# tczhangzhi/pytorch-distributed

Measured on AMD Instinct MI355X. Metric: ImageNet images/sec (ResNet-50 train step, whole job), higher is better.
Workload: dtype bf16; 1 GPU; model=resnet50, global_batch=3072, image_size=224, parallelism=dp1, style=ddp, hip_ext=True, hipgraph=False

## Files before the change

### amdtrain/models/resnet.py

```python

from __future__ import annotations

from typing import Callable, Dict, List, Optional, Type, Union

import torch
import torch.nn as nn

from ..ops import fused as OF


import os

from ..ops.conv import AmdConv2d, GradCell, ResidualGradTap
from ..ops.linear import AmdLinear


def _residual_fuse_enabled() -> bool:
    return os.environ.get("AMDTRAIN_RESFUSE", "1") == "1"


def conv3x3(in_planes: int, out_planes: int, stride: int = 1,
            groups: int = 1) -> nn.Conv2d:
    return AmdConv2d(in_planes, out_planes, kernel_size=3, stride=stride,
                     padding=1, groups=groups, bias=False)


def conv1x1(in_planes: int, out_planes: int, stride: int = 1) -> nn.Conv2d:
    return AmdConv2d(in_planes, out_planes, kernel_size=1, stride=stride,
                     bias=False)


class FusedBatchNorm2d(nn.BatchNorm2d):

    def forward(self, x: torch.Tensor) -> torch.Tensor:
        return OF.batch_norm(x, self, relu=False)

    def forward_relu(self, x: torch.Tensor) -> torch.Tensor:
        return OF.batch_norm(x, self, relu=True)


class BasicBlock(nn.Module):
    expansion = 1

    def __init__(self, inplanes: int, planes: int, stride: int = 1,
                 downsample: Optional[nn.Module] = None):
        super().__init__()
        self.conv1 = conv3x3(inplanes, planes, stride)
        self.bn1 = FusedBatchNorm2d(planes)
        self.relu = nn.ReLU(inplace=True)
        self.conv2 = conv3x3(planes, planes)
        self.bn2 = FusedBatchNorm2d(planes)
        self.downsample = downsample
        self.stride = stride

    def forward(self, x: torch.Tensor) -> torch.Tensor:
        identity = x
        cell = None
        if (self.training and x.is_cuda and torch.is_grad_enabled()
                and _residual_fuse_enabled()):
            cell = getattr(x, "_amdtrain_next_cell", None)
        out = self.bn1.forward_relu(self.conv1(x))
        out = self.conv2(out)
        if cell is not None:
            cell.armed = True
            tapped = ResidualGradTap.apply(x, cell)
            identity = self.downsample(tapped)                 if self.downsample is not None else tapped
        elif self.downsample is not None:
            identity = self.downsample(x)
        return OF.bn_add_relu(out, self.bn2, identity)


class Bottleneck(nn.Module):
    expansion = 4

    def __init__(self, inplanes: int, planes: int, stride: int = 1,
                 downsample: Optional[nn.Module] = None, groups: int = 1,
                 base_width: int = 64):
        super().__init__()
        width = int(planes * (base_width / 64.0)) * groups
        self.conv1 = conv1x1(inplanes, width)
        self.bn1 = FusedBatchNorm2d(width)
        self.conv2 = conv3x3(width, width, stride, groups)
        self.bn2 = FusedBatchNorm2d(width)
        self.conv3 = conv1x1(width, planes * self.expansion)
        self.bn3 = FusedBatchNorm2d(planes * self.expansion)
        self.relu = nn.ReLU(inplace=True)
        self.downsample = downsample
        self.stride = stride

    def forward(self, x: torch.Tensor) -> torch.Tensor:
        identity = x
        cell = None
        if (self.training and x.is_cuda and torch.is_grad_enabled()
                and _residual_fuse_enabled()):
            cell = getattr(x, "_amdtrain_next_cell", None)
        out = self.bn1.forward_relu(self.conv1(x))
        out = self.bn2.forward_relu(self.conv2(out))
        out = self.conv3(out)
        if cell is not None:
            cell.armed = True
            tapped = ResidualGradTap.apply(x, cell)
            identity = self.downsample(tapped)                 if self.downsample is not None else tapped
        elif self.downsample is not None:
            identity = self.downsample(x)
        return OF.bn_add_relu(out, self.bn3, identity)


class ResNet(nn.Module):
    def __init__(self, block: Type[Union[BasicBlock, Bottleneck]],
                 layers: List[int], num_classes: int = 1000,
                 zero_init_residual: bool = False, groups: int = 1,
                 width_per_group: int = 64):
        super().__init__()
        self.groups = groups
        self.base_width = width_per_group
        self.inplanes = 64
        self.conv1 = AmdConv2d(3, 64, kernel_size=7, stride=2, padding=3,
                               bias=False)
        self.bn1 = FusedBatchNorm2d(64)
        self.relu = nn.ReLU(inplace=True)
        self.maxpool = nn.MaxPool2d(kernel_size=3, stride=2, padding=1)
        self.layer1 = self._make_layer(block, 64, layers[0])
        self.layer2 = self._make_layer(block, 128, layers[1], stride=2)
        self.layer3 = self._make_layer(block, 256, layers[2], stride=2)
        self.layer4 = self._make_layer(block, 512, layers[3], stride=2)
        self.avgpool = nn.AdaptiveAvgPool2d((1, 1))
        self.fc = AmdLinear(512 * block.expansion, num_classes)

        for m in self.modules():
            if isinstance(m, nn.Conv2d):
                nn.init.kaiming_normal_(m.weight, mode="fan_out",
                                        nonlinearity="relu")
            elif isinstance(m, nn.BatchNorm2d):
                nn.init.constant_(m.weight, 1)
                nn.init.constant_(m.bias, 0)
        if zero_init_residual:
            for m in self.modules():
                if isinstance(m, Bottleneck):
                    nn.init.constant_(m.bn3.weight, 0)
                elif isinstance(m, BasicBlock):
                    nn.init.constant_(m.bn2.weight, 0)

    def _make_layer(self, block, planes: int, blocks: int,
                    stride: int = 1) -> nn.Sequential:
        downsample = None
        if stride != 1 or self.inplanes != planes * block.expansion:
            downsample = nn.Sequential(
                conv1x1(self.inplanes, planes * block.expansion, stride),
                FusedBatchNorm2d(planes * block.expansion),
            )
        kw = {}
        if block is Bottleneck:
            kw = dict(groups=self.groups, base_width=self.base_width)
        layers = [block(self.inplanes, planes, stride, downsample, **kw)]
        self.inplanes = planes * block.expansion
        for _ in range(1, blocks):
            layers.append(block(self.inplanes, planes, **kw))
        return nn.Sequential(*layers)

    def forward(self, x: torch.Tensor) -> torch.Tensor:
        x = self.bn1.forward_relu(self.conv1(x))
        x = OF.max_pool_3x3_s2(x)
        x = self.layer1(x)
        x = self.layer2(x)
        x = self.layer3(x)
        x = self.layer4(x)
        x = OF.global_avg_pool(x)
        x = torch.flatten(x, 1)
        return self.fc(x)


def resnet18(num_classes: int = 1000, **kw) -> ResNet:
    return ResNet(BasicBlock, [2, 2, 2, 2], num_classes=num_classes, **kw)


def resnet34(num_classes: int = 1000, **kw) -> ResNet:
    return ResNet(BasicBlock, [3, 4, 6, 3], num_classes=num_classes, **kw)


def resnet50(num_classes: int = 1000, **kw) -> ResNet:
    return ResNet(Bottleneck, [3, 4, 6, 3], num_classes=num_classes, **kw)


def resnet101(num_classes: int = 1000, **kw) -> ResNet:
    return ResNet(Bottleneck, [3, 4, 23, 3], num_classes=num_classes, **kw)


def resnet152(num_classes: int = 1000, **kw) -> ResNet:
    return ResNet(Bottleneck, [3, 8, 36, 3], num_classes=num_classes, **kw)


def resnext50_32x4d(num_classes: int = 1000, **kw) -> ResNet:
    return ResNet(Bottleneck, [3, 4, 6, 3], num_classes=num_classes,
                  groups=32, width_per_group=4, **kw)


def wide_resnet50_2(num_classes: int = 1000, **kw) -> ResNet:
    return ResNet(Bottleneck, [3, 4, 6, 3], num_classes=num_classes,
                  width_per_group=128, **kw)


_REGISTRY: Dict[str, Callable[..., nn.Module]] = {
    "resnet18": resnet18,
    "resnet34": resnet34,
    "resnet50": resnet50,
    "resnet101": resnet101,
    "resnet152": resnet152,
    "resnext50_32x4d": resnext50_32x4d,
    "wide_resnet50_2": wide_resnet50_2,
}


def model_names() -> List[str]:
    return sorted(_REGISTRY)


def build_model(arch: str, num_classes: int = 1000, **kw) -> nn.Module:
    if arch not in _REGISTRY:
        raise ValueError(f"unknown arch '{arch}'; choices: {model_names()}")
    return _REGISTRY[arch](num_classes=num_classes, **kw)
```

### amdtrain/ops/csrc/batchnorm.hip

```cpp
#include "common.h"

namespace {

template <typename T, int VEC, bool BWD, int MASK, bool WG, bool GO2>
__global__ void __launch_bounds__(AMD_TPB)
bn_reduce_kernel(const T* __restrict__ x, const T* __restrict__ go,
                 const T* __restrict__ goB, const T* __restrict__ y,
                 const float* __restrict__ mean,
                 const float* __restrict__ invstd,
                 const float* __restrict__ scale,
                 const float* __restrict__ shift, T* __restrict__ ghat_out,
                 float* __restrict__ out, long R, int C) {
  const int t = threadIdx.x;
  const int gpr = C / VEC;
  const long rows_per_block = (R + gridDim.x - 1) / gridDim.x;
  const long r0 = blockIdx.x * rows_per_block;
  const long r1 = min(r0 + rows_per_block, R);

  if (gpr <= AMD_TPB) {
    const int gc = t % gpr;
    const int phase = t / gpr;
    const int rstep = AMD_TPB / gpr;
    const int c0 = gc * VEC;
    float sa[VEC], sb[VEC];
#pragma unroll
    for (int k = 0; k < VEC; ++k) sa[k] = sb[k] = 0.f;
    float mk[VEC], ik[VEC], sck[VEC], shk[VEC];
    if (BWD) {
#pragma unroll
      for (int k = 0; k < VEC; ++k) {
        mk[k] = mean[c0 + k];
        ik[k] = invstd[c0 + k];
        if (MASK == 2) {
          sck[k] = scale[c0 + k];
          shk[k] = shift[c0 + k];
        }
      }
    }
    for (long r = r0 + phase; r < r1; r += rstep) {
      const long base = r * C + c0;
      Pack<T, VEC> xv = *(const Pack<T, VEC>*)(x + base);
      Pack<T, VEC> gv, gv2, yv, gh;
      unsigned int mbits = 0;
      if (BWD) {
        gv = *(const Pack<T, VEC>*)(go + base);
        if (GO2) gv2 = *(const Pack<T, VEC>*)(goB + base);
        if (MASK == 1) yv = *(const Pack<T, VEC>*)(y + base);
        if (MASK == 3)
          mbits = ((const unsigned char*)y)[base / VEC];
      }
#pragma unroll
      for (int k = 0; k < VEC; ++k) {
        float xe = to_f32(xv.v[k]);
        if (BWD) {
          float ge = to_f32(gv.v[k]);
          if (GO2) ge += to_f32(gv2.v[k]);
          if (MASK == 1 && to_f32(yv.v[k]) <= 0.f) ge = 0.f;
          if (MASK == 2 && sck[k] * xe + shk[k] <= 0.f) ge = 0.f;
          if (MASK == 3 && !(mbits & (1u << k))) ge = 0.f;
          sa[k] += ge;
          sb[k] += ge * (xe - mk[k]) * ik[k];
          if (WG) gh.v[k] = from_f32<T>(ge);
        } else {
          sa[k] += xe;
          sb[k] += xe * xe;
        }
      }
      if (BWD && WG) *(Pack<T, VEC>*)(ghat_out + base) = gh;
    }
    __shared__ float lds[AMD_TPB * VEC];
#pragma unroll
    for (int k = 0; k < VEC; ++k) lds[t * VEC + k] = sa[k];
    __syncthreads();
    if (phase == 0) {
      for (int ph = 1; ph < rstep; ++ph)
#pragma unroll
        for (int k = 0; k < VEC; ++k)
          sa[k] += lds[(ph * gpr + gc) * VEC + k];
    }
    __syncthreads();
#pragma unroll
    for (int k = 0; k < VEC; ++k) lds[t * VEC + k] = sb[k];
    __syncthreads();
    if (phase == 0) {
      for (int ph = 1; ph < rstep; ++ph)
#pragma unroll
        for (int k = 0; k < VEC; ++k)
          sb[k] += lds[(ph * gpr + gc) * VEC + k];
      float* part = out + (long)blockIdx.x * 2 * C;
#pragma unroll
      for (int k = 0; k < VEC; ++k) {
        part[c0 + k] = sa[k];
        part[C + c0 + k] = sb[k];
      }
    }
  } else {
    const int cpt = gpr / AMD_TPB;
    float sa[2][VEC], sb[2][VEC];
    float mk[2][VEC], ik[2][VEC], sck[2][VEC], shk[2][VEC];
#pragma unroll
    for (int j = 0; j < 2; ++j)
#pragma unroll
      for (int k = 0; k < VEC; ++k) {
        sa[j][k] = sb[j][k] = 0.f;
        if (BWD && j < cpt) {
          mk[j][k] = mean[(t + j * AMD_TPB) * VEC + k];
          ik[j][k] = invstd[(t + j * AMD_TPB) * VEC + k];
          if (MASK == 2) {
            sck[j][k] = scale[(t + j * AMD_TPB) * VEC + k];
            shk[j][k] = shift[(t + j * AMD_TPB) * VEC + k];
          }
        }
      }
    for (long r = r0; r < r1; ++r) {
      for (int j = 0; j < cpt; ++j) {
        const int c0 = (t + j * AMD_TPB) * VEC;
        const long base = r * C + c0;
        Pack<T, VEC> xv = *(const Pack<T, VEC>*)(x + base);
        Pack<T, VEC> gv, gv2, yv, gh;
        if (BWD) {
          gv = *(const Pack<T, VEC>*)(go + base);
          if (GO2) gv2 = *(const Pack<T, VEC>*)(goB + base);
          if (MASK == 1) yv = *(const Pack<T, VEC>*)(y + base);
        }
#pragma unroll
        for (int k = 0; k < VEC; ++k) {
          float xe = to_f32(xv.v[k]);
          if (BWD) {
            float ge = to_f32(gv.v[k]);
            if (GO2) ge += to_f32(gv2.v[k]);
            if (MASK == 1 && to_f32(yv.v[k]) <= 0.f) ge = 0.f;
            if (MASK == 2 && sck[j][k] * xe + shk[j][k] <= 0.f) ge = 0.f;
            sa[j][k] += ge;
            sb[j][k] += ge * (xe - mk[j][k]) * ik[j][k];
            if (WG) gh.v[k] = from_f32<T>(ge);
          } else {
            sa[j][k] += xe;
            sb[j][k] += xe * xe;
          }
        }
        if (BWD && WG) *(Pack<T, VEC>*)(ghat_out + base) = gh;
      }
    }
    float* part = out + (long)blockIdx.x * 2 * C;
    for (int j = 0; j < cpt; ++j) {
      const int c0 = (t + j * AMD_TPB) * VEC;
#pragma unroll
      for (int k = 0; k < VEC; ++k) {
        part[c0 + k] = sa[j][k];
        part[C + c0 + k] = sb[j][k];
      }
    }
  }
}

constexpr int BN_COLLAPSE = 32;

static inline int bn_collapse_slots(int nparts) {
  return nparts >= 2048 ? 4 * BN_COLLAPSE : BN_COLLAPSE;
}

__global__ void bn_collapse_partials_kernel(const float* __restrict__ in,
                                            float* __restrict__ out,
                                            int nparts, int twoC, int slots) {
  const int slot = blockIdx.x % slots;
  const int cblk = blockIdx.x / slots;
  const int c = cblk * AMD_TPB + threadIdx.x;
  if (c >= twoC) return;
  float acc = 0.f;
  for (int p = slot; p < nparts; p += slots)
    acc += in[(long)p * twoC + c];
  out[(long)slot * twoC + c] = acc;
}

__global__ void bn_finalize_train_kernel(
    const float* __restrict__ partials, int nparts,
    const float* __restrict__ w,
    const float* __restrict__ b, float* __restrict__ rm,
    float* __restrict__ rv, float* __restrict__ mean,
    float* __restrict__ invstd, float* __restrict__ scale,
    float* __restrict__ shift, long R, int C, float momentum, float eps) {
  const int c = blockIdx.x * 64 + (threadIdx.x & 63);
  const int sl = threadIdx.x >> 6;
  float s1 = 0.f, s2 = 0.f;
  if (c < C)
    for (int p = sl; p < nparts; p += 4) {
      s1 += partials[(long)p * 2 * C + c];
      s2 += partials[(long)p * 2 * C + C + c];
    }
  __shared__ float red[2][4][64];
  red[0][sl][threadIdx.x & 63] = s1;
  red[1][sl][threadIdx.x & 63] = s2;
  __syncthreads();
  if (sl != 0 || c >= C) return;
  s1 += red[0][1][threadIdx.x] + red[0][2][threadIdx.x] +
        red[0][3][threadIdx.x];
  s2 += red[1][1][threadIdx.x] + red[1][2][threadIdx.x] +
        red[1][3][threadIdx.x];
  float m = s1 / R;
  float var = fmaxf(s2 / R - m * m, 0.f);
  float is = rsqrtf(var + eps);
  mean[c] = m;
  invstd[c] = is;
  float unbiased = R > 1 ? var * (float)R / (float)(R - 1) : var;
  rm[c] = (1.f - momentum) * rm[c] + momentum * m;
  rv[c] = (1.f - momentum) * rv[c] + momentum * unbiased;
  float sc = w[c] * is;
  scale[c] = sc;
  shift[c] = b[c] - m * sc;
}

__global__ void bn_finalize_eval_kernel(
    const float* __restrict__ w, const float* __restrict__ b,
    const float* __restrict__ rm, const float* __restrict__ rv,
    float* __restrict__ scale, float* __restrict__ shift, int C, float eps) {
  int c = blockIdx.x * blockDim.x + threadIdx.x;
  if (c >= C) return;
  float is = rsqrtf(rv[c] + eps);
  float sc = w[c] * is;
  scale[c] = sc;
  shift[c] = b[c] - rm[c] * sc;
}

template <typename T, int VEC, bool RELU, bool HAS_ADD, bool POW2>
__global__ void __launch_bounds__(AMD_TPB)
bn_apply_kernel(const T* __restrict__ x, const T* __restrict__ z,
                T* __restrict__ y, unsigned char* __restrict__ mask,
                const float* __restrict__ scale,
                const float* __restrict__ shift, long total_vec, int C) {
  extern __shared__ float sm[];
  const int gpr = C / VEC;
  for (int c = threadIdx.x; c < C; c += blockDim.x) {
    sm[c] = scale[c];
    sm[C + c] = shift[c];
  }
  __syncthreads();
  const long stride = (long)gridDim.x * blockDim.x;
  for (long i = (long)blockIdx.x * blockDim.x + threadIdx.x; i < total_vec;
       i += 2 * stride) {
    const bool has2 = i + stride < total_vec;
    const long i2 = has2 ? i + stride : i;
    Pack<T, VEC> xv = *(const Pack<T, VEC>*)(x + i * VEC);
    Pack<T, VEC> xv2 = *(const Pack<T, VEC>*)(x + i2 * VEC);
    Pack<T, VEC> zv, zv2;
    if (HAS_ADD) {
      zv = *(const Pack<T, VEC>*)(z + i * VEC);
      zv2 = *(const Pack<T, VEC>*)(z + i2 * VEC);
    }
    const int c0 = (int)(POW2 ? (i & (gpr - 1)) : (i % gpr)) * VEC;
    const int c02 = (int)(POW2 ? (i2 & (gpr - 1)) : (i2 % gpr)) * VEC;
    Pack<T, VEC> yv, yv2;
    unsigned int mb = 0, mb2 = 0;
#pragma unroll
    for (int k = 0; k < VEC; ++k) {
      float v = sm[c0 + k] * to_f32(xv.v[k]) + sm[C + c0 + k];
      if (HAS_ADD) v += to_f32(zv.v[k]);
      if (RELU) {
        if (mask != nullptr && v > 0.f) mb |= 1u << k;
        v = fmaxf(v, 0.f);
      }
      yv.v[k] = from_f32<T>(v);
      float v2 = sm[c02 + k] * to_f32(xv2.v[k]) + sm[C + c02 + k];
      if (HAS_ADD) v2 += to_f32(zv2.v[k]);
      if (RELU) {
        if (mask != nullptr && v2 > 0.f) mb2 |= 1u << k;
        v2 = fmaxf(v2, 0.f);
      }
      yv2.v[k] = from_f32<T>(v2);
    }
    *(Pack<T, VEC>*)(y + i * VEC) = yv;
    if (has2) *(Pack<T, VEC>*)(y + i2 * VEC) = yv2;
    if (RELU && mask != nullptr) {
      mask[i] = (unsigned char)mb;
      if (has2) mask[i2] = (unsigned char)mb2;
    }
  }
}

__global__ void bn_bwd_finalize_kernel(
    const float* __restrict__ partials, int nparts,
    const float* __restrict__ w, const float* __restrict__ mean,
    const float* __restrict__ invstd, float* __restrict__ gw,
    float* __restrict__ gb, float* __restrict__ A, float* __restrict__ Bc,
    float* __restrict__ Dc, long R, int C) {
  const int c = blockIdx.x * 64 + (threadIdx.x & 63);
  const int sl = threadIdx.x >> 6;
  float sg = 0.f, sgx = 0.f;
  if (c < C)
    for (int p = sl; p < nparts; p += 4) {
      sg += partials[(long)p * 2 * C + c];
      sgx += partials[(long)p * 2 * C + C + c];
    }
  __shared__ float red[2][4][64];
  red[0][sl][threadIdx.x & 63] = sg;
  red[1][sl][threadIdx.x & 63] = sgx;
  __syncthreads();
  if (sl != 0 || c >= C) return;
  sg += red[0][1][threadIdx.x] + red[0][2][threadIdx.x] +
        red[0][3][threadIdx.x];
  sgx += red[1][1][threadIdx.x] + red[1][2][threadIdx.x] +
         red[1][3][threadIdx.x];
  gb[c] = sg;
  gw[c] = sgx;
  float a = w[c] * invstd[c];
  float bcoef = -a * invstd[c] * sgx / R;
  A[c] = a;
  Bc[c] = bcoef;
  Dc[c] = -a * sg / R - bcoef * mean[c];
}

template <typename T, int VEC, int MASK, bool WRITE_GHAT, bool POW2>
__global__ void __launch_bounds__(AMD_TPB)
bn_bwd_apply_kernel(const T* __restrict__ x, const T* __restrict__ go,
                    T* __restrict__ gx,
                    T* __restrict__ ghat_out, const float* __restrict__ A,
                    const float* __restrict__ Bc, const float* __restrict__ Dc,
                    const float* __restrict__ scale,
                    const float* __restrict__ shift, long total_vec, int C) {
  extern __shared__ float sm[];
  for (int c = threadIdx.x; c < C; c += blockDim.x) {
    sm[c] = A[c];
    sm[C + c] = Bc[c];
    sm[2 * C + c] = Dc[c];
    if (MASK == 2) {
      sm[3 * C + c] = scale[c];
      sm[4 * C + c] = shift[c];
    }
  }
  __syncthreads();
  const int gpr = C / VEC;
  const long stride = (long)gridDim.x * blockDim.x;
  for (long i = (long)blockIdx.x * blockDim.x + threadIdx.x; i < total_vec;
       i += 2 * stride) {
    const bool has2 = i + stride < total_vec;
    const long i2 = has2 ? i + stride : i;
    Pack<T, VEC> xv = *(const Pack<T, VEC>*)(x + i * VEC);
    Pack<T, VEC> gv = *(const Pack<T, VEC>*)(go + i * VEC);
    Pack<T, VEC> xv2 = *(const Pack<T, VEC>*)(x + i2 * VEC);
    Pack<T, VEC> gv2 = *(const Pack<T, VEC>*)(go + i2 * VEC);
    const int c0 = (int)(POW2 ? (i & (gpr - 1)) : (i % gpr)) * VEC;
    const int c02 = (int)(POW2 ? (i2 & (gpr - 1)) : (i2 % gpr)) * VEC;
    Pack<T, VEC> out, gh, out2, gh2;
#pragma unroll
    for (int k = 0; k < VEC; ++k) {
      float xe = to_f32(xv.v[k]);
      float ge = to_f32(gv.v[k]);
      if (MASK == 2 && sm[3 * C + c0 + k] * xe + sm[4 * C + c0 + k] <= 0.f)
        ge = 0.f;
      float v = sm[c0 + k] * ge + sm[C + c0 + k] * xe + sm[2 * C + c0 + k];
      out.v[k] = from_f32<T>(v);
      if (WRITE_GHAT) gh.v[k] = from_f32<T>(ge);
      float xe2 = to_f32(xv2.v[k]);
      float ge2 = to_f32(gv2.v[k]);
      if (MASK == 2 && sm[3 * C + c02 + k] * xe2 + sm[4 * C + c02 + k] <= 0.f)
        ge2 = 0.f;
      float v2 = sm[c02 + k] * ge2 + sm[C + c02 + k] * xe2 +
                 sm[2 * C + c02 + k];
      out2.v[k] = from_f32<T>(v2);
      if (WRITE_GHAT) gh2.v[k] = from_f32<T>(ge2);
    }
    *(Pack<T, VEC>*)(gx + i * VEC) = out;
    if (WRITE_GHAT) *(Pack<T, VEC>*)(ghat_out + i * VEC) = gh;
    if (has2) {
      *(Pack<T, VEC>*)(gx + i2 * VEC) = out2;
      if (WRITE_GHAT) *(Pack<T, VEC>*)(ghat_out + i2 * VEC) = gh2;
    }
  }
}


static void check_nhwc(const at::Tensor& x) {
  TORCH_CHECK(x.is_cuda() && x.dim() == 4, "expected 4D CUDA tensor");
  TORCH_CHECK(x.is_contiguous(at::MemoryFormat::ChannelsLast),
              "expected channels_last (NHWC) tensor");
}

template <typename F>
static void dispatch_vec(const at::Tensor& x, F fn) {
  int C = (int)x.size(1);
  AT_DISPATCH_FLOATING_TYPES_AND2(
      at::ScalarType::BFloat16, at::ScalarType::Half, x.scalar_type(), "bn",
      [&] {
        using devT = typename DevT<scalar_t>::type;
        constexpr int VEC = 16 / sizeof(devT);
        TORCH_CHECK(C % VEC == 0, "C must be a multiple of ", VEC);
        TORCH_CHECK((C & (C - 1)) == 0,
                    "C must be a power of two (apply-kernel fast path): ", C);
        TORCH_CHECK(C / VEC <= 2 * AMD_TPB, "C too large: ", C);
        fn((devT*)nullptr, std::integral_constant<int, VEC>{});
      });
}

static int bn_reduce_grid(long R, int C) {
  long rows_per_block = std::max<long>(1, R / 1536);
  return (int)std::min<long>((R + rows_per_block - 1) / rows_per_block, 1536);
}

}

std::vector<at::Tensor> batch_norm_fwd_train(
    at::Tensor x, at::Tensor weight, at::Tensor bias, at::Tensor running_mean,
    at::Tensor running_var, double momentum, double eps, bool relu,
    std::optional<at::Tensor> addend) {
  check_nhwc(x);
  const long N = x.size(0), C = x.size(1), H = x.size(2), W = x.size(3);
  const long R = N * H * W;
  auto opts = x.options().dtype(at::kFloat);
  const int rgrid = bn_reduce_grid(R, C);
  auto sums = at::empty({rgrid, 2 * C}, opts);
  auto mean = at::empty({C}, opts);
  auto invstd = at::empty({C}, opts);
  auto scale = at::empty({C}, opts);
  auto shift = at::empty({C}, opts);
  auto y = at::empty_like(x);
  at::Tensor mask;
  if (relu && addend)
    mask = at::empty({R * C / 4}, x.options().dtype(at::kByte));
  auto stream = at::cuda::getCurrentCUDAStream();

  dispatch_vec(x, [&](auto* tp, auto vec) {
    using devT = std::remove_pointer_t<decltype(tp)>;
    constexpr int VEC = decltype(vec)::value;
    bn_reduce_kernel<devT, VEC, false, 0, false, false>
        <<<rgrid, AMD_TPB, 0, stream>>>((const devT*)x.const_data_ptr(),
                                        nullptr, nullptr, nullptr, nullptr,
                                        nullptr, nullptr, nullptr, nullptr,
                                        sums.data_ptr<float>(), R, (int)C);
    CHECK_CUDA_OK();
    const int slots = bn_collapse_slots(rgrid);
    auto sums2 = at::empty({slots, 2 * C}, opts);
    {
      int cgrid = slots * (int)((2 * C + AMD_TPB - 1) / AMD_TPB);
      bn_collapse_partials_kernel<<<cgrid, AMD_TPB, 0, stream>>>(
          sums.data_ptr<float>(), sums2.data_ptr<float>(), rgrid,
          (int)(2 * C), slots);
      CHECK_CUDA_OK();
    }
    int fgrid = (int)((C + 63) / 64);
    bn_finalize_train_kernel<<<fgrid, AMD_TPB, 0, stream>>>(
        sums2.data_ptr<float>(), slots, weight.data_ptr<float>(),
        bias.data_ptr<float>(), running_mean.data_ptr<float>(),
        running_var.data_ptr<float>(), mean.data_ptr<float>(),
        invstd.data_ptr<float>(), scale.data_ptr<float>(),
        shift.data_ptr<float>(), R, (int)C, (float)momentum, (float)eps);
    CHECK_CUDA_OK();
    long total_vec = R * C / VEC;
    int agrid = amd_grid(total_vec);
    size_t smem = 2 * C * sizeof(float);
    const devT* zp =
        addend ? (const devT*)addend->const_data_ptr() : nullptr;
#define APPLY(RELU_, ADD_)                                                  \
  bn_apply_kernel<devT, VEC, RELU_, ADD_, true>                             \
      <<<agrid, AMD_TPB, smem, stream>>>(                                   \
          (const devT*)x.const_data_ptr(), zp, (devT*)y.data_ptr(),         \
          mask.defined() ? mask.data_ptr<unsigned char>() : nullptr,        \
          scale.data_ptr<float>(), shift.data_ptr<float>(),     \
          total_vec, (int)C)
    if (relu && addend) APPLY(true, true);
    else if (relu) APPLY(true, false);
    else if (addend) APPLY(false, true);
    else APPLY(false, false);
#undef APPLY
    CHECK_CUDA_OK();
  });
  if (!mask.defined()) mask = at::empty({0}, x.options().dtype(at::kByte));
  return {y, mean, invstd, scale, shift, mask};
}

std::vector<at::Tensor> batch_norm_fwd_train_from_parts(
    at::Tensor x, at::Tensor parts, at::Tensor weight, at::Tensor bias,
    at::Tensor running_mean, at::Tensor running_var, double momentum,
    double eps, bool relu, std::optional<at::Tensor> addend) {
  check_nhwc(x);
  const long C = x.size(1);
  const long R = x.numel() / C;
  TORCH_CHECK(parts.size(1) == 2 * C, "parts must be [nparts][2C]");
  const int nparts = (int)parts.size(0);
  auto opts = x.options().dtype(at::kFloat);
  auto mean = at::empty({C}, opts);
  auto invstd = at::empty({C}, opts);
  auto scale = at::empty({C}, opts);
  auto shift = at::empty({C}, opts);
  auto y = at::empty_like(x);
  at::Tensor mask;
  if (relu && addend)
    mask = at::empty({R * C / 4}, x.options().dtype(at::kByte));
  auto stream = at::cuda::getCurrentCUDAStream();

  const int slots = bn_collapse_slots(nparts);
  auto sums2 = at::empty({slots, 2 * C}, opts);
  {
    int cgrid = slots * (int)((2 * C + AMD_TPB - 1) / AMD_TPB);
    bn_collapse_partials_kernel<<<cgrid, AMD_TPB, 0, stream>>>(
        parts.data_ptr<float>(), sums2.data_ptr<float>(), nparts,
        (int)(2 * C), slots);
    CHECK_CUDA_OK();
  }
  int fgrid = (int)((C + 63) / 64);
  bn_finalize_train_kernel<<<fgrid, AMD_TPB, 0, stream>>>(
      sums2.data_ptr<float>(), slots, weight.data_ptr<float>(),
      bias.data_ptr<float>(), running_mean.data_ptr<float>(),
      running_var.data_ptr<float>(), mean.data_ptr<float>(),
      invstd.data_ptr<float>(), scale.data_ptr<float>(),
      shift.data_ptr<float>(), R, (int)C, (float)momentum, (float)eps);
  CHECK_CUDA_OK();
  dispatch_vec(x, [&](auto* tp, auto vec) {
    using devT = std::remove_pointer_t<decltype(tp)>;
    constexpr int VEC = decltype(vec)::value;
    long total_vec = R * C / VEC;
    int agrid = amd_grid(total_vec);
    size_t smem = 2 * C * sizeof(float);
    const devT* zp =
        addend ? (const devT*)addend->const_data_ptr() : nullptr;
#define APPLY2(RELU_, ADD_)                                                 \
  bn_apply_kernel<devT, VEC, RELU_, ADD_, true>                             \
      <<<agrid, AMD_TPB, smem, stream>>>(                                   \
          (const devT*)x.const_data_ptr(), zp, (devT*)y.data_ptr(),         \
          mask.defined() ? mask.data_ptr<unsigned char>() : nullptr,        \
          scale.data_ptr<float>(), shift.data_ptr<float>(),                 \
          total_vec, (int)C)
    if (relu && addend) APPLY2(true, true);
    else if (relu) APPLY2(true, false);
    else if (addend) APPLY2(false, true);
    else APPLY2(false, false);
#undef APPLY2
    CHECK_CUDA_OK();
  });
  if (!mask.defined()) mask = at::empty({0}, x.options().dtype(at::kByte));
  return {y, mean, invstd, scale, shift, mask};
}

at::Tensor batch_norm_fwd_eval(at::Tensor x, at::Tensor weight,
                               at::Tensor bias, at::Tensor running_mean,
                               at::Tensor running_var, double eps, bool relu,
                               std::optional<at::Tensor> addend) {
  check_nhwc(x);
  const long C = x.size(1);
  const long R = x.numel() / C;
  auto opts = x.options().dtype(at::kFloat);
  auto scale = at::empty({C}, opts);
  auto shift = at::empty({C}, opts);
  auto y = at::empty_like(x);
  at::Tensor mask;
  auto stream = at::cuda::getCurrentCUDAStream();
  int fgrid = (int)((C + AMD_TPB - 1) / AMD_TPB);
  bn_finalize_eval_kernel<<<fgrid, AMD_TPB, 0, stream>>>(
      weight.data_ptr<float>(), bias.data_ptr<float>(),
      running_mean.data_ptr<float>(), running_var.data_ptr<float>(),
      scale.data_ptr<float>(), shift.data_ptr<float>(), (int)C, (float)eps);
  CHECK_CUDA_OK();
  dispatch_vec(x, [&](auto* tp, auto vec) {
    using devT = std::remove_pointer_t<decltype(tp)>;
    constexpr int VEC = decltype(vec)::value;
    long total_vec = R * C / VEC;
    int agrid = amd_grid(total_vec);
    size_t smem = 2 * C * sizeof(float);
    const devT* zp =
        addend ? (const devT*)addend->const_data_ptr() : nullptr;
#define APPLY(RELU_, ADD_)                                                  \
  bn_apply_kernel<devT, VEC, RELU_, ADD_, true>                             \
      <<<agrid, AMD_TPB, smem, stream>>>(                                   \
          (const devT*)x.const_data_ptr(), zp, (devT*)y.data_ptr(),         \
          mask.defined() ? mask.data_ptr<unsigned char>() : nullptr,        \
          scale.data_ptr<float>(), shift.data_ptr<float>(),     \
          total_vec, (int)C)
    if (relu && addend) APPLY(true, true);
    else if (relu) APPLY(true, false);
    else if (addend) APPLY(false, true);
    else APPLY(false, false);
#undef APPLY
    CHECK_CUDA_OK();
  });
  return y;
}

std::vector<at::Tensor> batch_norm_bwd(at::Tensor x, at::Tensor grad_out,
                                       at::Tensor y, at::Tensor weight,
                                       at::Tensor mean, at::Tensor invstd,
                                       bool relu, bool need_ghat,
                                       std::optional<at::Tensor> scale,
                                       std::optional<at::Tensor> shift,
                                       std::optional<at::Tensor> grad_out2,
                                       std::optional<at::Tensor> relu_mask) {
  check_nhwc(x);
  check_nhwc(grad_out);
  const long C = x.size(1);
  const long R = x.numel() / C;
  auto opts = x.options().dtype(at::kFloat);
  const int rgrid = bn_reduce_grid(R, C);
  auto sums = at::empty({rgrid, 2 * C}, opts);
  auto gw = at::empty({C}, opts);
  auto gb = at::empty({C}, opts);
  auto A = at::empty({C}, opts);
  auto Bc = at::empty({C}, opts);
  auto Dc = at::empty({C}, opts);
  auto gx = at::empty_like(x);
  const bool affine_mask = relu && !need_ghat && scale && shift;
  const bool mask_y = relu && (!affine_mask || grad_out2.has_value());
  at::Tensor ghat;
  if (mask_y || grad_out2) ghat = at::empty_like(grad_out);
  auto stream = at::cuda::getCurrentCUDAStream();

  dispatch_vec(x, [&](auto* tp, auto vec) {
    using devT = std::remove_pointer_t<decltype(tp)>;
    constexpr int VEC = decltype(vec)::value;
    const float* scp = affine_mask ? scale->data_ptr<float>() : nullptr;
    const float* shp = affine_mask ? shift->data_ptr<float>() : nullptr;
    const devT* go2p = grad_out2
        ? (const devT*)grad_out2->const_data_ptr() : nullptr;
#define REDUCE(MASK_, WG_, GO2_)                                            \
  bn_reduce_kernel<devT, VEC, true, MASK_, WG_, GO2_>                       \
      <<<rgrid, AMD_TPB, 0, stream>>>(                                      \
          (const devT*)x.const_data_ptr(),                                  \
          (const devT*)grad_out.const_data_ptr(), go2p,                     \
          (const devT*)y.const_data_ptr(), mean.data_ptr<float>(),          \
          invstd.data_ptr<float>(), scp, shp,                               \
          WG_ ? (devT*)ghat.data_ptr() : nullptr,                           \
          sums.data_ptr<float>(), R, (int)C)
#define REDUCE3(GO2_)                                                       \
  bn_reduce_kernel<devT, VEC, true, 3, true, GO2_>                          \
      <<<rgrid, AMD_TPB, 0, stream>>>(                                      \
          (const devT*)x.const_data_ptr(),                                  \
          (const devT*)grad_out.const_data_ptr(), go2p,                     \
          (const devT*)mkp, mean.data_ptr<float>(),                         \
          invstd.data_ptr<float>(), scp, shp,                               \
          (devT*)ghat.data_ptr(),                                           \
          sums.data_ptr<float>(), R, (int)C)
    const unsigned char* mkp = (relu_mask && relu_mask->numel())
        ? relu_mask->data_ptr<unsigned char>() : nullptr;
    if (mask_y && mkp && go2p) REDUCE3(true);
    else if (mask_y && mkp) REDUCE3(false);
    else if (mask_y && go2p) REDUCE(1, true, true);
    else if (mask_y) REDUCE(1, true, false);
    else if (affine_mask) REDUCE(2, false, false);
    else if (go2p) REDUCE(0, true, true);
    else REDUCE(0, false, false);
#undef REDUCE
#undef REDUCE3
    CHECK_CUDA_OK();
    const int slots = bn_collapse_slots(rgrid);
    auto sums2 = at::empty({slots, 2 * C}, opts);
    {
      int cgrid = slots * (int)((2 * C + AMD_TPB - 1) / AMD_TPB);
      bn_collapse_partials_kernel<<<cgrid, AMD_TPB, 0, stream>>>(
          sums.data_ptr<float>(), sums2.data_ptr<float>(), rgrid,
          (int)(2 * C), slots);
      CHECK_CUDA_OK();
    }
    int fgrid = (int)((C + 63) / 64);
    bn_bwd_finalize_kernel<<<fgrid, AMD_TPB, 0, stream>>>(
        sums2.data_ptr<float>(), slots, weight.data_ptr<float>(),
        mean.data_ptr<float>(), invstd.data_ptr<float>(),
        gw.data_ptr<float>(), gb.data_ptr<float>(), A.data_ptr<float>(),
        Bc.data_ptr<float>(), Dc.data_ptr<float>(), R, (int)C);
    CHECK_CUDA_OK();
    long total_vec = R * C / VEC;
    int agrid = amd_grid(total_vec);
    size_t smem = (affine_mask ? 5 : 3) * C * sizeof(float);
    const devT* go_in = ghat.defined()
                            ? (const devT*)ghat.const_data_ptr()
                            : (const devT*)grad_out.const_data_ptr();
#define BAPPLY(MASK_)                                                       \
  bn_bwd_apply_kernel<devT, VEC, MASK_, false, true>                        \
      <<<agrid, AMD_TPB, smem, stream>>>(                                   \
          (const devT*)x.const_data_ptr(), go_in, (devT*)gx.data_ptr(),     \
          nullptr, A.data_ptr<float>(), Bc.data_ptr<float>(),               \
          Dc.data_ptr<float>(), scp, shp, total_vec, (int)C)
    if (affine_mask) BAPPLY(2);
    else BAPPLY(0);
#undef BAPPLY
    CHECK_CUDA_OK();
  });
  if (!ghat.defined()) ghat = grad_out;
  return {gx, gw, gb, ghat};
}
```

### amdtrain/ops/csrc/ext.cpp

```cpp
#include <torch/extension.h>

#include <optional>
#include <vector>

void multi_tensor_sgd(std::vector<at::Tensor> params,
                      std::vector<at::Tensor> grads,
                      std::vector<at::Tensor> momenta, double lr,
                      double momentum, double weight_decay, bool nesterov,
                      bool first, bool zero_grad);

std::vector<at::Tensor> cross_entropy_fwd(at::Tensor logits, at::Tensor target);
at::Tensor cross_entropy_bwd(at::Tensor logits, at::Tensor target,
                             at::Tensor lse, at::Tensor upstream);

at::Tensor normalize_u8(at::Tensor x, std::vector<double> mean,
                        std::vector<double> std_, long dtype_code);
at::Tensor topk_ranks(at::Tensor logits, at::Tensor target);
at::Tensor scatter_rows_x2(at::Tensor src2d, long Nn, long H, long W,
                           long Hs, long Ws);
void multi_tensor_scale_check(std::vector<at::Tensor> tensors, double scale,
                              at::Tensor found_inf);
void multi_tensor_cast(std::vector<at::Tensor> src,
                       std::vector<at::Tensor> dst);

std::vector<at::Tensor> batch_norm_fwd_train(
    at::Tensor x, at::Tensor weight, at::Tensor bias, at::Tensor running_mean,
    at::Tensor running_var, double momentum, double eps, bool relu,
    std::optional<at::Tensor> addend);
std::vector<at::Tensor> batch_norm_fwd_train_from_parts(
    at::Tensor x, at::Tensor parts, at::Tensor weight, at::Tensor bias,
    at::Tensor running_mean, at::Tensor running_var, double momentum,
    double eps, bool relu, std::optional<at::Tensor> addend);
at::Tensor batch_norm_fwd_eval(at::Tensor x, at::Tensor weight,
                               at::Tensor bias, at::Tensor running_mean,
                               at::Tensor running_var, double eps, bool relu,
                               std::optional<at::Tensor> addend);
std::vector<at::Tensor> batch_norm_bwd(at::Tensor x, at::Tensor grad_out,
                                       at::Tensor y, at::Tensor weight,
                                       at::Tensor mean, at::Tensor invstd,
                                       bool relu, bool need_ghat,
                                       std::optional<at::Tensor> scale,
                                       std::optional<at::Tensor> shift,
                                       std::optional<at::Tensor> grad_out2,
                                       std::optional<at::Tensor> relu_mask);

at::Tensor gemm_bt(at::Tensor A, at::Tensor B, bool f32_out,
                   std::optional<at::Tensor> addend,
                   std::optional<at::Tensor> bias);
at::Tensor gemm_tn(at::Tensor dY, at::Tensor X, long msplit);
at::Tensor gemm_bt_strided(at::Tensor A, at::Tensor B, long Nn, long H,
                           long W, long stride);
at::Tensor gemm_tn_strided(at::Tensor dY, at::Tensor X, long Nn, long H,
                           long W, long stride);
at::Tensor transpose_2d(at::Tensor x);

at::Tensor conv3x3_fwd(at::Tensor x2d, long Nn, long H, long W, long stride,
                       at::Tensor w2d);
std::vector<at::Tensor> conv3x3_fwd_stats(at::Tensor x2d, long Nn, long H,
                                          long W, long stride,
                                          at::Tensor w2d, bool banded);
std::vector<at::Tensor> gemm_bt_stats(at::Tensor A, at::Tensor B);

at::Tensor gemm_bt_8p(at::Tensor A, at::Tensor B);
at::Tensor gemm_bt_8p3(at::Tensor A, at::Tensor B);
at::Tensor conv3x3_8p(at::Tensor A2d, long Nn, long H, long W, long stride,
                      at::Tensor w2d, bool dgrad);
at::Tensor conv3x3_dgrad(at::Tensor dy2d, long Nn, long H, long W,
                         long stride, at::Tensor w2d, bool banded);
at::Tensor conv3x3_wgrad(at::Tensor dy2d, at::Tensor x2d, long Nn, long H,
                         long W, long stride);

at::Tensor tn2_wgrad(at::Tensor dY, at::Tensor X, long taps, long Nn, long H,
                     long W, long stride, long gmode, long kh, long kw,
                     long pad);
at::Tensor tn2_wgrad_banded(at::Tensor dY, at::Tensor X, long Nn, long H,
                            long W, long stride);
at::Tensor tr16_probe(at::Tensor in);

at::Tensor conv_generic_fwd(at::Tensor x2d, long Nn, long H, long W, long KH,
                            long KW, long stride, long pad, at::Tensor w2);
at::Tensor conv_generic_wgrad(at::Tensor dy2d, at::Tensor x2d, long Nn,
                              long H, long W, long KH, long KW, long stride,
                              long pad);
at::Tensor conv_generic_dgrad(at::Tensor dy2d, at::Tensor w2p, long Nn,
                              long H, long W, long KH, long KW, long stride,
                              long pad);

std::vector<at::Tensor> max_pool_3x3_s2_fwd(at::Tensor x);
at::Tensor max_pool_3x3_s2_bwd(at::Tensor grad_y, at::Tensor idx, long H,
                               long W);
at::Tensor global_avg_pool_fwd(at::Tensor x);
at::Tensor global_avg_pool_bwd(at::Tensor grad_y, long H, long W);

PYBIND11_MODULE(TORCH_EXTENSION_NAME, m) {
  m.doc() = "amdtrain hand-written gfx950 (CDNA4) HIP kernels";
  m.def("multi_tensor_sgd", &multi_tensor_sgd, "fused multi-tensor SGD");
  m.def("cross_entropy_fwd", &cross_entropy_fwd);
  m.def("cross_entropy_bwd", &cross_entropy_bwd);
  m.def("normalize_u8", &normalize_u8);
  m.def("topk_ranks", &topk_ranks);
  m.def("scatter_rows_x2", &scatter_rows_x2);
  m.def("multi_tensor_scale_check", &multi_tensor_scale_check);
  m.def("multi_tensor_cast", &multi_tensor_cast);
  m.def("batch_norm_fwd_train", &batch_norm_fwd_train,
        py::arg("x"), py::arg("weight"), py::arg("bias"),
        py::arg("running_mean"), py::arg("running_var"), py::arg("momentum"),
        py::arg("eps"), py::arg("relu"),
        py::arg("addend") = std::nullopt);
  m.def("batch_norm_fwd_train_from_parts", &batch_norm_fwd_train_from_parts,
        py::arg("x"), py::arg("parts"), py::arg("weight"), py::arg("bias"),
        py::arg("running_mean"), py::arg("running_var"), py::arg("momentum"),
        py::arg("eps"), py::arg("relu"), py::arg("addend") = std::nullopt);
  m.def("batch_norm_fwd_eval", &batch_norm_fwd_eval,
        py::arg("x"), py::arg("weight"), py::arg("bias"),
        py::arg("running_mean"), py::arg("running_var"), py::arg("eps"),
        py::arg("relu"), py::arg("addend") = std::nullopt);
  m.def("batch_norm_bwd", &batch_norm_bwd, py::arg("x"), py::arg("grad_out"),
        py::arg("y"), py::arg("weight"), py::arg("mean"), py::arg("invstd"),
        py::arg("relu"), py::arg("need_ghat"),
        py::arg("scale") = std::nullopt, py::arg("shift") = std::nullopt,
        py::arg("grad_out2") = std::nullopt,
        py::arg("relu_mask") = std::nullopt);
  m.def("gemm_bt", &gemm_bt, py::arg("A"), py::arg("B"),
        py::arg("f32_out") = false, py::arg("addend") = std::nullopt,
        py::arg("bias") = std::nullopt);
  m.def("gemm_tn", &gemm_tn, py::arg("dY"), py::arg("X"),
        py::arg("msplit") = 0);
  m.def("gemm_bt_strided", &gemm_bt_strided);
  m.def("gemm_tn_strided", &gemm_tn_strided);
  m.def("transpose_2d", &transpose_2d);
  m.def("conv3x3_fwd", &conv3x3_fwd);
  m.def("conv3x3_fwd_stats", &conv3x3_fwd_stats, py::arg("x2d"),
        py::arg("Nn"), py::arg("H"), py::arg("W"), py::arg("stride"),
        py::arg("w2d"), py::arg("banded") = false);
  m.def("gemm_bt_stats", &gemm_bt_stats);
  m.def("gemm_bt_8p", &gemm_bt_8p);
  m.def("gemm_bt_8p3", &gemm_bt_8p3);
  m.def("conv3x3_8p", &conv3x3_8p);
  m.def("conv3x3_dgrad", &conv3x3_dgrad, py::arg("dy2d"), py::arg("Nn"),
        py::arg("H"), py::arg("W"), py::arg("stride"), py::arg("w2d"),
        py::arg("banded") = false);
  m.def("conv3x3_wgrad", &conv3x3_wgrad);
  m.def("tn2_wgrad", &tn2_wgrad, py::arg("dY"), py::arg("X"),
        py::arg("taps") = 1, py::arg("Nn") = 0, py::arg("H") = 0,
        py::arg("W") = 0, py::arg("stride") = 1, py::arg("gmode") = 0,
        py::arg("kh") = 3, py::arg("kw") = 3, py::arg("pad") = 1);
  m.def("tn2_wgrad_banded", &tn2_wgrad_banded);
  m.def("tr16_probe", &tr16_probe);
  m.def("conv_generic_fwd", &conv_generic_fwd);
  m.def("conv_generic_wgrad", &conv_generic_wgrad);
  m.def("conv_generic_dgrad", &conv_generic_dgrad);
  m.def("max_pool_3x3_s2_fwd", &max_pool_3x3_s2_fwd);
  m.def("max_pool_3x3_s2_bwd", &max_pool_3x3_s2_bwd);
  m.def("global_avg_pool_fwd", &global_avg_pool_fwd);
  m.def("global_avg_pool_bwd", &global_avg_pool_bwd);
}
```

### amdtrain/ops/csrc/pool.hip

```cpp
#include "common.h"

namespace {

template <typename T, int VEC>
__global__ void __launch_bounds__(AMD_TPB)
maxpool_fwd_kernel(const T* __restrict__ x, T* __restrict__ y,
                   unsigned char* __restrict__ idx, long N, int H, int W,
                   int C, int Ho, int Wo) {
  const int gpr = C / VEC;
  const long total = N * Ho * Wo * gpr;
  for (long i = (long)blockIdx.x * blockDim.x + threadIdx.x; i < total;
       i += (long)gridDim.x * blockDim.x) {
    long t = i;
    const int gc = (int)(t % gpr); t /= gpr;
    const int wo = (int)(t % Wo); t /= Wo;
    const int ho = (int)(t % Ho); t /= Ho;
    const long n = t;
    const int c0 = gc * VEC;

    float best[VEC];
    unsigned char bidx[VEC];
#pragma unroll
    for (int k = 0; k < VEC; ++k) {
      best[k] = -INFINITY;
      bidx[k] = 255;
    }
    const int h0 = ho * 2 - 1, w0 = wo * 2 - 1;
#pragma unroll
    for (int kh = 0; kh < 3; ++kh) {
      const int h = h0 + kh;
      if (h < 0 || h >= H) continue;
#pragma unroll
      for (int kw = 0; kw < 3; ++kw) {
        const int w = w0 + kw;
        if (w < 0 || w >= W) continue;
        const long base = ((n * H + h) * W + w) * C + c0;
        Pack<T, VEC> xv = *(const Pack<T, VEC>*)(x + base);
#pragma unroll
        for (int k = 0; k < VEC; ++k) {
          float v = to_f32(xv.v[k]);
          if (v > best[k]) {
            best[k] = v;
            bidx[k] = (unsigned char)(kh * 3 + kw);
          }
        }
      }
    }
    const long obase = ((n * Ho + ho) * Wo + wo) * C + c0;
    Pack<T, VEC> yv;
    Pack<unsigned char, VEC> iv;
#pragma unroll
    for (int k = 0; k < VEC; ++k) {
      yv.v[k] = from_f32<T>(best[k]);
      iv.v[k] = bidx[k];
    }
    *(Pack<T, VEC>*)(y + obase) = yv;
    *(Pack<unsigned char, VEC>*)(idx + obase) = iv;
  }
}

template <typename T, int VEC>
__global__ void __launch_bounds__(AMD_TPB)
maxpool_bwd_kernel(const T* __restrict__ gy, const unsigned char* __restrict__ idx,
                   T* __restrict__ gx, long N, int H, int W, int C, int Ho,
                   int Wo) {
  const int gpr = C / VEC;
  const long total = N * H * W * gpr;
  for (long i = (long)blockIdx.x * blockDim.x + threadIdx.x; i < total;
       i += (long)gridDim.x * blockDim.x) {
    long t = i;
    const int gc = (int)(t % gpr); t /= gpr;
    const int w = (int)(t % W); t /= W;
    const int h = (int)(t % H); t /= H;
    const long n = t;
    const int c0 = gc * VEC;

    float acc[VEC];
#pragma unroll
    for (int k = 0; k < VEC; ++k) acc[k] = 0.f;
    const int ho_lo = max(0, (h - 1 + 1) / 2);
    const int ho_hi = min(Ho - 1, (h + 1) / 2);
    const int wo_lo = max(0, (w - 1 + 1) / 2);
    const int wo_hi = min(Wo - 1, (w + 1) / 2);
    for (int ho = ho_lo; ho <= ho_hi; ++ho) {
      const int kh = h - (ho * 2 - 1);
      for (int wo = wo_lo; wo <= wo_hi; ++wo) {
        const int kw = w - (wo * 2 - 1);
        const unsigned char code = (unsigned char)(kh * 3 + kw);
        const long obase = ((n * Ho + ho) * Wo + wo) * C + c0;
        Pack<unsigned char, VEC> iv =
            *(const Pack<unsigned char, VEC>*)(idx + obase);
        Pack<T, VEC> gv = *(const Pack<T, VEC>*)(gy + obase);
#pragma unroll
        for (int k = 0; k < VEC; ++k)
          if (iv.v[k] == code) acc[k] += to_f32(gv.v[k]);
      }
    }
    const long base = ((n * H + h) * W + w) * C + c0;
    Pack<T, VEC> out;
#pragma unroll
    for (int k = 0; k < VEC; ++k) out.v[k] = from_f32<T>(acc[k]);
    *(Pack<T, VEC>*)(gx + base) = out;
  }
}

template <typename T, int VEC>
__global__ void __launch_bounds__(AMD_TPB)
gap_fwd_kernel(const T* __restrict__ x, T* __restrict__ y, long N, int HW,
               int C) {
  const int gpr = C / VEC;
  const long total = N * gpr;
  const float inv = 1.f / HW;
  for (long i = (long)blockIdx.x * blockDim.x + threadIdx.x; i < total;
       i += (long)gridDim.x * blockDim.x) {
    const long n = i / gpr;
    const int c0 = (int)(i % gpr) * VEC;
    float acc[VEC];
#pragma unroll
    for (int k = 0; k < VEC; ++k) acc[k] = 0.f;
    const T* xp = x + n * (long)HW * C + c0;
    for (int r = 0; r < HW; ++r) {
      Pack<T, VEC> xv = *(const Pack<T, VEC>*)(xp + (long)r * C);
#pragma unroll
      for (int k = 0; k < VEC; ++k) acc[k] += to_f32(xv.v[k]);
    }
    Pack<T, VEC> yv;
#pragma unroll
    for (int k = 0; k < VEC; ++k) yv.v[k] = from_f32<T>(acc[k] * inv);
    *(Pack<T, VEC>*)(y + n * C + c0) = yv;
  }
}

template <typename T, int VEC>
__global__ void __launch_bounds__(AMD_TPB)
gap_bwd_kernel(const T* __restrict__ gy, T* __restrict__ gx, long N, int HW,
               int C) {
  const int gpr = C / VEC;
  const long total = N * (long)HW * gpr;
  const float inv = 1.f / HW;
  for (long i = (long)blockIdx.x * blockDim.x + threadIdx.x; i < total;
       i += (long)gridDim.x * blockDim.x) {
    const long row = i / gpr;
    const long n = row / HW;
    const int c0 = (int)(i % gpr) * VEC;
    Pack<T, VEC> gv = *(const Pack<T, VEC>*)(gy + n * C + c0);
    Pack<T, VEC> out;
#pragma unroll
    for (int k = 0; k < VEC; ++k)
      out.v[k] = from_f32<T>(to_f32(gv.v[k]) * inv);
    *(Pack<T, VEC>*)(gx + row * C + c0) = out;
  }
}

static void check_nhwc4(const at::Tensor& x) {
  TORCH_CHECK(x.is_cuda() && x.dim() == 4 &&
                  x.is_contiguous(at::MemoryFormat::ChannelsLast),
              "expected NHWC CUDA tensor");
}

}

std::vector<at::Tensor> max_pool_3x3_s2_fwd(at::Tensor x) {
  check_nhwc4(x);
  const long N = x.size(0), C = x.size(1), H = x.size(2), W = x.size(3);
  const long Ho = (H + 2 - 3) / 2 + 1, Wo = (W + 2 - 3) / 2 + 1;
  auto y = at::empty({N, C, Ho, Wo},
                     x.options().memory_format(at::MemoryFormat::ChannelsLast));
  auto idx = at::empty({N, C, Ho, Wo}, x.options()
                                           .dtype(at::kByte)
                                           .memory_format(
                                               at::MemoryFormat::ChannelsLast));
  auto stream = at::cuda::getCurrentCUDAStream();
  AT_DISPATCH_FLOATING_TYPES_AND2(
      at::ScalarType::BFloat16, at::ScalarType::Half, x.scalar_type(),
      "maxpool_fwd", [&] {
        using devT = typename DevT<scalar_t>::type;
        constexpr int VEC = 16 / sizeof(devT);
        TORCH_CHECK(C % VEC == 0);
        long total = N * Ho * Wo * (C / VEC);
        maxpool_fwd_kernel<devT, VEC>
            <<<amd_grid(total), AMD_TPB, 0, stream>>>(
                (const devT*)x.const_data_ptr(), (devT*)y.data_ptr(),
                (unsigned char*)idx.data_ptr(), N, (int)H, (int)W, (int)C,
                (int)Ho, (int)Wo);
        CHECK_CUDA_OK();
      });
  return {y, idx};
}

at::Tensor max_pool_3x3_s2_bwd(at::Tensor grad_y, at::Tensor idx, long H,
                               long W) {
  check_nhwc4(grad_y);
  const long N = grad_y.size(0), C = grad_y.size(1), Ho = grad_y.size(2),
             Wo = grad_y.size(3);
  auto gx = at::empty({N, C, H, W},
                      grad_y.options().memory_format(
                          at::MemoryFormat::ChannelsLast));
  auto stream = at::cuda::getCurrentCUDAStream();
  AT_DISPATCH_FLOATING_TYPES_AND2(
      at::ScalarType::BFloat16, at::ScalarType::Half, grad_y.scalar_type(),
      "maxpool_bwd", [&] {
        using devT = typename DevT<scalar_t>::type;
        constexpr int VEC = 16 / sizeof(devT);
        long total = N * H * W * (C / VEC);
        maxpool_bwd_kernel<devT, VEC>
            <<<amd_grid(total), AMD_TPB, 0, stream>>>(
                (const devT*)grad_y.const_data_ptr(),
                (const unsigned char*)idx.const_data_ptr(),
                (devT*)gx.data_ptr(), N, (int)H, (int)W, (int)C, (int)Ho,
                (int)Wo);
        CHECK_CUDA_OK();
      });
  return gx;
}

at::Tensor global_avg_pool_fwd(at::Tensor x) {
  check_nhwc4(x);
  const long N = x.size(0), C = x.size(1), H = x.size(2), W = x.size(3);
  auto y = at::empty({N, C, 1, 1}, x.options());
  auto stream = at::cuda::getCurrentCUDAStream();
  AT_DISPATCH_FLOATING_TYPES_AND2(
      at::ScalarType::BFloat16, at::ScalarType::Half, x.scalar_type(),
      "gap_fwd", [&] {
        using devT = typename DevT<scalar_t>::type;
        constexpr int VEC = 16 / sizeof(devT);
        long total = N * (C / VEC);
        gap_fwd_kernel<devT, VEC><<<amd_grid(total), AMD_TPB, 0, stream>>>(
            (const devT*)x.const_data_ptr(), (devT*)y.data_ptr(), N,
            (int)(H * W), (int)C);
        CHECK_CUDA_OK();
      });
  return y;
}

at::Tensor global_avg_pool_bwd(at::Tensor grad_y, long H, long W) {
  TORCH_CHECK(grad_y.is_cuda());
  auto g = grad_y.contiguous();
  const long N = g.size(0), C = g.size(1);
  auto gx = at::empty({N, C, H, W},
                      g.options().memory_format(
                          at::MemoryFormat::ChannelsLast));
  auto stream = at::cuda::getCurrentCUDAStream();
  AT_DISPATCH_FLOATING_TYPES_AND2(
      at::ScalarType::BFloat16, at::ScalarType::Half, g.scalar_type(),
      "gap_bwd", [&] {
        using devT = typename DevT<scalar_t>::type;
        constexpr int VEC = 16 / sizeof(devT);
        long total = N * H * W * (C / VEC);
        gap_bwd_kernel<devT, VEC><<<amd_grid(total), AMD_TPB, 0, stream>>>(
            (const devT*)g.const_data_ptr(), (devT*)gx.data_ptr(), N,
            (int)(H * W), (int)C);
        CHECK_CUDA_OK();
      });
  return gx;
}
```

### amdtrain/ops/fused.py

```python

from __future__ import annotations

from typing import Optional

import torch
import torch.nn.functional as F

from ._ext import require_ext, use_ext_for
from .conv import GradCell

__all__ = ["batch_norm", "bn_add_relu", "max_pool_3x3_s2", "global_avg_pool"]


class _BNFunction(torch.autograd.Function):

    @staticmethod
    def forward(ctx, x, weight, bias, running_mean, running_var,
                momentum, eps, relu, addend, parts, res_cell=None):
        e = require_ext()
        if parts is not None:
            y, mean, invstd, scale, shift, mask = \
                e.batch_norm_fwd_train_from_parts(
                    x, parts, weight, bias, running_mean, running_var,
                    float(momentum), float(eps), bool(relu), addend)
        else:
            y, mean, invstd, scale, shift, mask = e.batch_norm_fwd_train(
                x, weight, bias, running_mean, running_var,
                float(momentum), float(eps), bool(relu), addend)
        ctx.save_for_backward(x, y, weight, mean, invstd, scale, shift,
                              mask)
        ctx.relu = bool(relu)
        ctx.has_addend = addend is not None
        ctx.res_cell = res_cell
        return y

    @staticmethod
    def backward(ctx, grad_out):
        x, y, weight, mean, invstd, scale, shift, mask = ctx.saved_tensors
        e = require_ext()
        go2 = None
        cell = getattr(ctx, "res_cell", None)
        if cell is not None and cell.g is not None:
            go2 = cell.g.contiguous(memory_format=torch.channels_last)
            cell.g = None
        grad_x, grad_w, grad_b, ghat = e.batch_norm_bwd(
            x, grad_out.contiguous(memory_format=torch.channels_last),
            y, weight, mean, invstd, ctx.relu, ctx.has_addend,
            scale, shift, go2, mask)
        grad_addend = ghat if ctx.has_addend else None
        return (grad_x, grad_w, grad_b, None, None, None, None, None,
                grad_addend, None, None)


def _bn_torch(x: torch.Tensor, bn, relu: bool,
              addend: Optional[torch.Tensor]) -> torch.Tensor:
    y = F.batch_norm(
        x, bn.running_mean, bn.running_var, bn.weight, bn.bias,
        bn.training or not bn.track_running_stats,
        bn.momentum if bn.momentum is not None else 0.0, bn.eps)
    if addend is not None:
        y = y + addend
    if relu:
        y = F.relu(y, inplace=True)
    return y


def batch_norm(x: torch.Tensor, bn, relu: bool = False,
               addend: Optional[torch.Tensor] = None) -> torch.Tensor:
    if bn.training and bn.track_running_stats and bn.num_batches_tracked is not None:
        bn.num_batches_tracked.add_(1)
    C = x.size(1)
    if use_ext_for(x) and (C & (C - 1)) == 0:
        parts = getattr(x, "_amdtrain_bn_stats", None) if bn.training else None
        xc = x.contiguous(memory_format=torch.channels_last)
        ac = None if addend is None else addend.contiguous(memory_format=torch.channels_last)
        if bn.training:
            cell = GradCell() if (relu and ac is not None) else None
            out = _BNFunction.apply(xc, bn.weight, bn.bias, bn.running_mean,
                                    bn.running_var, bn.momentum, bn.eps,
                                    relu, ac, parts, cell)
            if cell is not None:
                out._amdtrain_next_cell = cell
            return out
        return require_ext().batch_norm_fwd_eval(
            xc, bn.weight, bn.bias, bn.running_mean, bn.running_var,
            float(bn.eps), bool(relu), ac)
    return _bn_torch(x, bn, relu, addend)


def bn_add_relu(x: torch.Tensor, bn, addend: torch.Tensor) -> torch.Tensor:
    return batch_norm(x, bn, relu=True, addend=addend)


class _MaxPool3x3S2(torch.autograd.Function):
    @staticmethod
    def forward(ctx, x):
        e = require_ext()
        y, idx = e.max_pool_3x3_s2_fwd(x)
        ctx.save_for_backward(idx)
        ctx.in_shape = x.shape
        return y

    @staticmethod
    def backward(ctx, grad_out):
        (idx,) = ctx.saved_tensors
        e = require_ext()
        n, c, h, w = ctx.in_shape
        gx = e.max_pool_3x3_s2_bwd(
            grad_out.contiguous(memory_format=torch.channels_last), idx,
            int(h), int(w))
        return gx


def max_pool_3x3_s2(x: torch.Tensor) -> torch.Tensor:
    if use_ext_for(x):
        return _MaxPool3x3S2.apply(x.contiguous(memory_format=torch.channels_last))
    return F.max_pool2d(x, kernel_size=3, stride=2, padding=1)


class _GlobalAvgPool(torch.autograd.Function):
    @staticmethod
    def forward(ctx, x):
        e = require_ext()
        y = e.global_avg_pool_fwd(x)
        ctx.in_shape = x.shape
        return y

    @staticmethod
    def backward(ctx, grad_out):
        e = require_ext()
        n, c, h, w = ctx.in_shape
        return e.global_avg_pool_bwd(grad_out.contiguous(), int(h), int(w))


def global_avg_pool(x: torch.Tensor) -> torch.Tensor:
    if use_ext_for(x):
        return _GlobalAvgPool.apply(x.contiguous(memory_format=torch.channels_last))
    return F.adaptive_avg_pool2d(x, (1, 1))
```

Before: 9864 images/sec.

## Fuse downsample BN into residual BN-add-ReLU and stem BN-ReLU into maxpool

Adds a dual batch-norm path that normalizes the downsample shortcut inside the main branch's BN+add+ReLU kernel, so the normalized shortcut tensor is never materialized. The backward pass computes both BN gradients together. Separately, the stem BN+ReLU is folded into the maxpool forward, which skips writing the full-resolution activation, and the BN is recomputed in backward. This cuts memory traffic on large activations, at the cost of more kernel variants, recomputation, and heavier register use in the reduce kernels.

```diff
diff --git a/amdtrain/models/resnet.py b/amdtrain/models/resnet.py
--- a/amdtrain/models/resnet.py
+++ b/amdtrain/models/resnet.py
@@ -37,6 +37,17 @@
 
     def forward_relu(self, x: torch.Tensor) -> torch.Tensor:
         return OF.batch_norm(x, self, relu=True)
+
+
+def _shortcut_tail(out: torch.Tensor, bn: FusedBatchNorm2d,
+                   downsample: nn.Module, x: torch.Tensor) -> torch.Tensor:
+    if (bn.training and isinstance(downsample, nn.Sequential)
+            and len(downsample) == 2
+            and isinstance(downsample[0], AmdConv2d)
+            and isinstance(downsample[1], FusedBatchNorm2d)):
+        return OF.bn_add_relu_downsample(out, bn, downsample[0](x),
+                                         downsample[1])
+    return OF.bn_add_relu(out, bn, downsample(x))
 
 
 class BasicBlock(nn.Module):
@@ -63,10 +74,9 @@
         out = self.conv2(out)
         if cell is not None:
             cell.armed = True
-            tapped = ResidualGradTap.apply(x, cell)
-            identity = self.downsample(tapped)                 if self.downsample is not None else tapped
-        elif self.downsample is not None:
-            identity = self.downsample(x)
+            identity = ResidualGradTap.apply(x, cell)
+        if self.downsample is not None:
+            return _shortcut_tail(out, self.bn2, self.downsample, identity)
         return OF.bn_add_relu(out, self.bn2, identity)
 
 
@@ -99,10 +109,9 @@
         out = self.conv3(out)
         if cell is not None:
             cell.armed = True
-            tapped = ResidualGradTap.apply(x, cell)
-            identity = self.downsample(tapped)                 if self.downsample is not None else tapped
-        elif self.downsample is not None:
-            identity = self.downsample(x)
+            identity = ResidualGradTap.apply(x, cell)
+        if self.downsample is not None:
+            return _shortcut_tail(out, self.bn3, self.downsample, identity)
         return OF.bn_add_relu(out, self.bn3, identity)
 
 
@@ -159,8 +168,7 @@
         return nn.Sequential(*layers)
 
     def forward(self, x: torch.Tensor) -> torch.Tensor:
-        x = self.bn1.forward_relu(self.conv1(x))
-        x = OF.max_pool_3x3_s2(x)
+        x = OF.bn_relu_max_pool(self.conv1(x), self.bn1)
         x = self.layer1(x)
         x = self.layer2(x)
         x = self.layer3(x)
diff --git a/amdtrain/ops/csrc/batchnorm.hip b/amdtrain/ops/csrc/batchnorm.hip
--- a/amdtrain/ops/csrc/batchnorm.hip
+++ b/amdtrain/ops/csrc/batchnorm.hip
@@ -2,7 +2,16 @@
 
 namespace {
 
-template <typename T, int VEC, bool BWD, int MASK, bool WG, bool GO2>
+template <typename T>
+struct BNDualSide {
+  const T* x = nullptr;
+  const float* mean = nullptr;
+  const float* invstd = nullptr;
+  float* out = nullptr;
+};
+
+template <typename T, int VEC, bool BWD, int MASK, bool WG, bool GO2,
+          bool DUAL = false>
 __global__ void __launch_bounds__(AMD_TPB)
 bn_reduce_kernel(const T* __restrict__ x, const T* __restrict__ go,
                  const T* __restrict__ goB, const T* __restrict__ y,
@@ -10,7 +19,9 @@
                  const float* __restrict__ invstd,
                  const float* __restrict__ scale,
                  const float* __restrict__ shift, T* __restrict__ ghat_out,
-                 float* __restrict__ out, long R, int C) {
+                 float* __restrict__ out, long R, int C,
+                 BNDualSide<T> ds = {}) {
+  static_assert(!DUAL || (BWD && WG), "DUAL rides the ghat-writing bwd pass");
   const int t = threadIdx.x;
   const int gpr = C / VEC;
   const long rows_per_block = (R + gridDim.x - 1) / gridDim.x;
@@ -26,6 +37,7 @@
 #pragma unroll
     for (int k = 0; k < VEC; ++k) sa[k] = sb[k] = 0.f;
     float mk[VEC], ik[VEC], sck[VEC], shk[VEC];
+    float sda[VEC], sdb[VEC], mdk[VEC], idk[VEC];
     if (BWD) {
 #pragma unroll
       for (int k = 0; k < VEC; ++k) {
@@ -35,15 +47,21 @@
           sck[k] = scale[c0 + k];
           shk[k] = shift[c0 + k];
         }
+        if (DUAL) {
+          sda[k] = sdb[k] = 0.f;
+          mdk[k] = ds.mean[c0 + k];
+          idk[k] = ds.invstd[c0 + k];
+        }
       }
     }
     for (long r = r0 + phase; r < r1; r += rstep) {
       const long base = r * C + c0;
       Pack<T, VEC> xv = *(const Pack<T, VEC>*)(x + base);
-      Pack<T, VEC> gv, gv2, yv, gh;
+      Pack<T, VEC> gv, gv2, yv, gh, dv;
       unsigned int mbits = 0;
       if (BWD) {
         gv = *(const Pack<T, VEC>*)(go + base);
+        if (DUAL) dv = *(const Pack<T, VEC>*)(ds.x + base);
         if (GO2) gv2 = *(const Pack<T, VEC>*)(goB + base);
         if (MASK == 1) yv = *(const Pack<T, VEC>*)(y + base);
         if (MASK == 3)
@@ -61,6 +79,11 @@
           sa[k] += ge;
           sb[k] += ge * (xe - mk[k]) * ik[k];
           if (WG) gh.v[k] = from_f32<T>(ge);
+          if (DUAL) {
+            const float gr = to_f32(gh.v[k]);
+            sda[k] += gr;
+            sdb[k] += gr * (to_f32(dv.v[k]) - mdk[k]) * idk[k];
+          }
         } else {
           sa[k] += xe;
           sb[k] += xe * xe;
@@ -69,29 +92,38 @@
       if (BWD && WG) *(Pack<T, VEC>*)(ghat_out + base) = gh;
     }
     __shared__ float lds[AMD_TPB * VEC];
-#pragma unroll
-    for (int k = 0; k < VEC; ++k) lds[t * VEC + k] = sa[k];
-    __syncthreads();
+    auto fold = [&](float(&s)[VEC]) {
+#pragma unroll
+      for (int k = 0; k < VEC; ++k) lds[t * VEC + k] = s[k];
+      __syncthreads();
+      if (phase == 0) {
+        for (int ph = 1; ph < rstep; ++ph)
+#pragma unroll
+          for (int k = 0; k < VEC; ++k)
+            s[k] += lds[(ph * gpr + gc) * VEC + k];
+      }
+      __syncthreads();
+    };
+    fold(sa);
+    fold(sb);
+    if (DUAL) {
+      fold(sda);
+      fold(sdb);
+    }
     if (phase == 0) {
-      for (int ph = 1; ph < rstep; ++ph)
-#pragma unroll
-        for (int k = 0; k < VEC; ++k)
-          sa[k] += lds[(ph * gpr + gc) * VEC + k];
-    }
-    __syncthreads();
-#pragma unroll
-    for (int k = 0; k < VEC; ++k) lds[t * VEC + k] = sb[k];
-    __syncthreads();
-    if (phase == 0) {
-      for (int ph = 1; ph < rstep; ++ph)
-#pragma unroll
-        for (int k = 0; k < VEC; ++k)
-          sb[k] += lds[(ph * gpr + gc) * VEC + k];
       float* part = out + (long)blockIdx.x * 2 * C;
 #pragma unroll
       for (int k = 0; k < VEC; ++k) {
         part[c0 + k] = sa[k];
         part[C + c0 + k] = sb[k];
+      }
+      if (DUAL) {
+        float* partd = ds.out + (long)blockIdx.x * 2 * C;
+#pragma unroll
+        for (int k = 0; k < VEC; ++k) {
+          partd[c0 + k] = sda[k];
+          partd[C + c0 + k] = sdb[k];
+        }
       }
     }
   } else {
@@ -118,10 +150,13 @@
         const long base = r * C + c0;
         Pack<T, VEC> xv = *(const Pack<T, VEC>*)(x + base);
         Pack<T, VEC> gv, gv2, yv, gh;
+        unsigned int mbits = 0;
         if (BWD) {
           gv = *(const Pack<T, VEC>*)(go + base);
           if (GO2) gv2 = *(const Pack<T, VEC>*)(goB + base);
           if (MASK == 1) yv = *(const Pack<T, VEC>*)(y + base);
+          if (MASK == 3)
+            mbits = ((const unsigned char*)y)[base / VEC];
         }
 #pragma unroll
         for (int k = 0; k < VEC; ++k) {
@@ -131,6 +166,7 @@
             if (GO2) ge += to_f32(gv2.v[k]);
             if (MASK == 1 && to_f32(yv.v[k]) <= 0.f) ge = 0.f;
             if (MASK == 2 && sck[j][k] * xe + shk[j][k] <= 0.f) ge = 0.f;
+            if (MASK == 3 && !(mbits & (1u << k))) ge = 0.f;
             sa[j][k] += ge;
             sb[j][k] += ge * (xe - mk[j][k]) * ik[j][k];
             if (WG) gh.v[k] = from_f32<T>(ge);
@@ -222,20 +258,37 @@
   shift[c] = b[c] - rm[c] * sc;
 }
 
-template <typename T, int VEC, bool RELU, bool HAS_ADD, bool POW2>
+template <typename T, int VEC, bool RELU, bool HAS_ADD, bool POW2,
+          bool DUAL = false>
 __global__ void __launch_bounds__(AMD_TPB)
 bn_apply_kernel(const T* __restrict__ x, const T* __restrict__ z,
                 T* __restrict__ y, unsigned char* __restrict__ mask,
                 const float* __restrict__ scale,
-                const float* __restrict__ shift, long total_vec, int C) {
+                const float* __restrict__ shift, long total_vec, int C,
+                const float* __restrict__ scale_d = nullptr,
+                const float* __restrict__ shift_d = nullptr) {
+  static_assert(!DUAL || (HAS_ADD && POW2), "DUAL normalizes the addend");
   extern __shared__ float sm[];
   const int gpr = C / VEC;
-  for (int c = threadIdx.x; c < C; c += blockDim.x) {
-    sm[c] = scale[c];
-    sm[C + c] = shift[c];
+  const long stride = (long)gridDim.x * blockDim.x;
+  float rs[VEC], rb[VEC], rsd[VEC], rbd[VEC];
+  if (DUAL) {
+    const int cf =
+        (int)(((long)blockIdx.x * blockDim.x + threadIdx.x) & (gpr - 1)) * VEC;
+#pragma unroll
+    for (int k = 0; k < VEC; ++k) {
+      rs[k] = scale[cf + k];
+      rb[k] = shift[cf + k];
+      rsd[k] = scale_d[cf + k];
+      rbd[k] = shift_d[cf + k];
+    }
+  } else {
+    for (int c = threadIdx.x; c < C; c += blockDim.x) {
+      sm[c] = scale[c];
+      sm[C + c] = shift[c];
+    }
+    __syncthreads();
   }
-  __syncthreads();
-  const long stride = (long)gridDim.x * blockDim.x;
   for (long i = (long)blockIdx.x * blockDim.x + threadIdx.x; i < total_vec;
        i += 2 * stride) {
     const bool has2 = i + stride < total_vec;
@@ -253,15 +306,25 @@
     unsigned int mb = 0, mb2 = 0;
 #pragma unroll
     for (int k = 0; k < VEC; ++k) {
-      float v = sm[c0 + k] * to_f32(xv.v[k]) + sm[C + c0 + k];
-      if (HAS_ADD) v += to_f32(zv.v[k]);
+      float v = DUAL ? rs[k] * to_f32(xv.v[k]) + rb[k]
+                     : sm[c0 + k] * to_f32(xv.v[k]) + sm[C + c0 + k];
+      if (HAS_ADD) {
+        float ze = to_f32(zv.v[k]);
+        if (DUAL) ze = to_f32(from_f32<T>(rsd[k] * ze + rbd[k]));
+        v += ze;
+      }
       if (RELU) {
         if (mask != nullptr && v > 0.f) mb |= 1u << k;
         v = fmaxf(v, 0.f);
       }
       yv.v[k] = from_f32<T>(v);
-      float v2 = sm[c02 + k] * to_f32(xv2.v[k]) + sm[C + c02 + k];
-      if (HAS_ADD) v2 += to_f32(zv2.v[k]);
+      float v2 = DUAL ? rs[k] * to_f32(xv2.v[k]) + rb[k]
+                      : sm[c02 + k] * to_f32(xv2.v[k]) + sm[C + c02 + k];
+      if (HAS_ADD) {
+        float ze2 = to_f32(zv2.v[k]);
+        if (DUAL) ze2 = to_f32(from_f32<T>(rsd[k] * ze2 + rbd[k]));
+        v2 += ze2;
+      }
       if (RELU) {
         if (mask != nullptr && v2 > 0.f) mb2 |= 1u << k;
         v2 = fmaxf(v2, 0.f);
@@ -309,14 +372,74 @@
   Dc[c] = -a * sg / R - bcoef * mean[c];
 }
 
-template <typename T, int VEC, int MASK, bool WRITE_GHAT, bool POW2>
+template <typename T>
+struct BNDualBwdSide {
+  const T* x = nullptr;
+  T* gx = nullptr;
+  const float* A = nullptr;
+  const float* Bc = nullptr;
+  const float* Dc = nullptr;
+};
+
+template <typename T, int VEC, int MASK, bool WRITE_GHAT, bool POW2,
+          bool DUAL = false>
 __global__ void __launch_bounds__(AMD_TPB)
 bn_bwd_apply_kernel(const T* __restrict__ x, const T* __restrict__ go,
                     T* __restrict__ gx,
                     T* __restrict__ ghat_out, const float* __restrict__ A,
                     const float* __restrict__ Bc, const float* __restrict__ Dc,
                     const float* __restrict__ scale,
-                    const float* __restrict__ shift, long total_vec, int C) {
+                    const float* __restrict__ shift, long total_vec, int C,
+                    BNDualBwdSide<T> ds = {}) {
+  static_assert(!DUAL || (MASK == 0 && POW2 && !WRITE_GHAT),
+                "DUAL consumes the materialized ghat");
+  const int gpr = C / VEC;
+  const long stride = (long)gridDim.x * blockDim.x;
+  if (DUAL) {
+    const long i0 = (long)blockIdx.x * blockDim.x + threadIdx.x;
+    const int c0 = (int)(i0 & (gpr - 1)) * VEC;
+    float a3[VEC], b3[VEC], d3[VEC], ad[VEC], bd[VEC], dd[VEC];
+#pragma unroll
+    for (int k = 0; k < VEC; ++k) {
+      a3[k] = A[c0 + k];
+      b3[k] = Bc[c0 + k];
+      d3[k] = Dc[c0 + k];
+      ad[k] = ds.A[c0 + k];
+      bd[k] = ds.Bc[c0 + k];
+      dd[k] = ds.Dc[c0 + k];
+    }
+    for (long i = i0; i < total_vec; i += 2 * stride) {
+      const bool has2 = i + stride < total_vec;
+      const long i2 = has2 ? i + stride : i;
+      Pack<T, VEC> xv = *(const Pack<T, VEC>*)(x + i * VEC);
+      Pack<T, VEC> dv = *(const Pack<T, VEC>*)(ds.x + i * VEC);
+      Pack<T, VEC> gv = *(const Pack<T, VEC>*)(go + i * VEC);
+      Pack<T, VEC> xv2 = *(const Pack<T, VEC>*)(x + i2 * VEC);
+      Pack<T, VEC> dv2 = *(const Pack<T, VEC>*)(ds.x + i2 * VEC);
+      Pack<T, VEC> gv2 = *(const Pack<T, VEC>*)(go + i2 * VEC);
+      Pack<T, VEC> out, dout, out2, dout2;
+#pragma unroll
+      for (int k = 0; k < VEC; ++k) {
+        float ge = to_f32(gv.v[k]);
+        float v = a3[k] * ge + b3[k] * to_f32(xv.v[k]) + d3[k];
+        out.v[k] = from_f32<T>(v);
+        float w = ad[k] * ge + bd[k] * to_f32(dv.v[k]) + dd[k];
+        dout.v[k] = from_f32<T>(w);
+        float ge2 = to_f32(gv2.v[k]);
+        float v2 = a3[k] * ge2 + b3[k] * to_f32(xv2.v[k]) + d3[k];
+        out2.v[k] = from_f32<T>(v2);
+        float w2 = ad[k] * ge2 + bd[k] * to_f32(dv2.v[k]) + dd[k];
+        dout2.v[k] = from_f32<T>(w2);
+      }
+      *(Pack<T, VEC>*)(gx + i * VEC) = out;
+      *(Pack<T, VEC>*)(ds.gx + i * VEC) = dout;
+      if (has2) {
+        *(Pack<T, VEC>*)(gx + i2 * VEC) = out2;
+        *(Pack<T, VEC>*)(ds.gx + i2 * VEC) = dout2;
+      }
+    }
+    return;
+  }
   extern __shared__ float sm[];
   for (int c = threadIdx.x; c < C; c += blockDim.x) {
     sm[c] = A[c];
@@ -328,8 +451,6 @@
     }
   }
   __syncthreads();
-  const int gpr = C / VEC;
-  const long stride = (long)gridDim.x * blockDim.x;
   for (long i = (long)blockIdx.x * blockDim.x + threadIdx.x; i < total_vec;
        i += 2 * stride) {
     const bool has2 = i + stride < total_vec;
@@ -396,6 +517,110 @@
   return (int)std::min<long>((R + rows_per_block - 1) / rows_per_block, 1536);
 }
 
+static at::Tensor bn_collapse(const at::Tensor& parts, long C,
+                              hipStream_t stream) {
+  const int nparts = (int)parts.size(0);
+  const int slots = bn_collapse_slots(nparts);
+  auto sums2 = at::empty({slots, 2 * C}, parts.options());
+  int cgrid = slots * (int)((2 * C + AMD_TPB - 1) / AMD_TPB);
+  bn_collapse_partials_kernel<<<cgrid, AMD_TPB, 0, stream>>>(
+      parts.data_ptr<float>(), sums2.data_ptr<float>(), nparts, (int)(2 * C),
+      slots);
+  CHECK_CUDA_OK();
+  return sums2;
+}
+
+struct BNTrainStats {
+  at::Tensor mean, invstd, scale, shift;
+};
+
+static BNTrainStats bn_train_stats(const at::Tensor& x,
+                                   const std::optional<at::Tensor>& parts,
+                                   const at::Tensor& weight,
+                                   const at::Tensor& bias,
+                                   at::Tensor& running_mean,
+                                   at::Tensor& running_var, double momentum,
+                                   double eps) {
+  const long C = x.size(1);
+  const long R = x.numel() / C;
+  auto opts = x.options().dtype(at::kFloat);
+  auto stream = at::cuda::getCurrentCUDAStream();
+  at::Tensor sums;
+  if (parts) {
+    TORCH_CHECK(parts->size(1) == 2 * C, "parts must be [nparts][2C]");
+    sums = *parts;
+  } else {
+    const int rgrid = bn_reduce_grid(R, C);
+    sums = at::empty({rgrid, 2 * C}, opts);
+    dispatch_vec(x, [&](auto* tp, auto vec) {
+      using devT = std::remove_pointer_t<decltype(tp)>;
+      constexpr int VEC = decltype(vec)::value;
+      bn_reduce_kernel<devT, VEC, false, 0, false, false>
+          <<<rgrid, AMD_TPB, 0, stream>>>((const devT*)x.const_data_ptr(),
+                                          nullptr, nullptr, nullptr, nullptr,
+                                          nullptr, nullptr, nullptr, nullptr,
+                                          sums.data_ptr<float>(), R, (int)C);
+      CHECK_CUDA_OK();
+    });
+  }
+  auto sums2 = bn_collapse(sums, C, stream);
+  BNTrainStats s{at::empty({C}, opts), at::empty({C}, opts),
+                 at::empty({C}, opts), at::empty({C}, opts)};
+  int fgrid = (int)((C + 63) / 64);
+  bn_finalize_train_kernel<<<fgrid, AMD_TPB, 0, stream>>>(
+      sums2.data_ptr<float>(), (int)sums2.size(0), weight.data_ptr<float>(),
+      bias.data_ptr<float>(), running_mean.data_ptr<float>(),
+      running_var.data_ptr<float>(), s.mean.data_ptr<float>(),
+      s.invstd.data_ptr<float>(), s.scale.data_ptr<float>(),
+      s.shift.data_ptr<float>(), R, (int)C, (float)momentum, (float)eps);
+  CHECK_CUDA_OK();
+  return s;
+}
+
+struct BNBwdCoeffs {
+  at::Tensor gw, gb, A, Bc, Dc;
+};
+
+static BNBwdCoeffs bn_bwd_coeffs(const at::Tensor& sums,
+                                 const at::Tensor& weight,
+                                 const at::Tensor& mean,
+                                 const at::Tensor& invstd, long R, long C) {
+  auto stream = at::cuda::getCurrentCUDAStream();
+  auto opts = sums.options();
+  auto sums2 = bn_collapse(sums, C, stream);
+  BNBwdCoeffs k{at::empty({C}, opts), at::empty({C}, opts),
+                at::empty({C}, opts), at::empty({C}, opts),
+                at::empty({C}, opts)};
+  int fgrid = (int)((C + 63) / 64);
+  bn_bwd_finalize_kernel<<<fgrid, AMD_TPB, 0, stream>>>(
+      sums2.data_ptr<float>(), (int)sums2.size(0), weight.data_ptr<float>(),
+      mean.data_ptr<float>(), invstd.data_ptr<float>(),
+      k.gw.data_ptr<float>(), k.gb.data_ptr<float>(), k.A.data_ptr<float>(),
+      k.Bc.data_ptr<float>(), k.Dc.data_ptr<float>(), R, (int)C);
+  CHECK_CUDA_OK();
+  return k;
+}
+
+static void check_dual(const at::Tensor& x3, const at::Tensor& x_d) {
+  check_nhwc(x3);
+  check_nhwc(x_d);
+  TORCH_CHECK(x3.sizes() == x_d.sizes() &&
+                  x3.scalar_type() == x_d.scalar_type(),
+              "dual BN tail: x3 and x_d must match in shape and dtype");
+  TORCH_CHECK(x3.size(1) * (long)x3.element_size() / 16 <= AMD_TPB,
+              "dual BN tail: C too wide for the register path: ", x3.size(1));
+}
+
+}
+
+std::vector<at::Tensor> batch_norm_train_stats(
+    at::Tensor x, std::optional<at::Tensor> parts, at::Tensor weight,
+    at::Tensor bias, at::Tensor running_mean, at::Tensor running_var,
+    double momentum, double eps) {
+  check_nhwc(x);
+  auto s = bn_train_stats(x, parts, weight, bias, running_mean, running_var,
+                          momentum, eps);
+  return {s.mean, s.invstd, s.scale, s.shift};
 }
 
 std::vector<at::Tensor> batch_norm_fwd_train(
@@ -405,45 +630,19 @@
   check_nhwc(x);
   const long N = x.size(0), C = x.size(1), H = x.size(2), W = x.size(3);
   const long R = N * H * W;
-  auto opts = x.options().dtype(at::kFloat);
-  const int rgrid = bn_reduce_grid(R, C);
-  auto sums = at::empty({rgrid, 2 * C}, opts);
-  auto mean = at::empty({C}, opts);
-  auto invstd = at::empty({C}, opts);
-  auto scale = at::empty({C}, opts);
-  auto shift = at::empty({C}, opts);
   auto y = at::empty_like(x);
   at::Tensor mask;
   if (relu && addend)
     mask = at::empty({R * C / 4}, x.options().dtype(at::kByte));
   auto stream = at::cuda::getCurrentCUDAStream();
+  auto st = bn_train_stats(x, std::nullopt, weight, bias, running_mean,
+                           running_var, momentum, eps);
+  auto &mean = st.mean, &invstd = st.invstd, &scale = st.scale,
+       &shift = st.shift;
 
   dispatch_vec(x, [&](auto* tp, auto vec) {
     using devT = std::remove_pointer_t<decltype(tp)>;
     constexpr int VEC = decltype(vec)::value;
-    bn_reduce_kernel<devT, VEC, false, 0, false, false>
-        <<<rgrid, AMD_TPB, 0, stream>>>((const devT*)x.const_data_ptr(),
-                                        nullptr, nullptr, nullptr, nullptr,
-                                        nullptr, nullptr, nullptr, nullptr,
-                                        sums.data_ptr<float>(), R, (int)C);
-    CHECK_CUDA_OK();
-    const int slots = bn_collapse_slots(rgrid);
-    auto sums2 = at::empty({slots, 2 * C}, opts);
-    {
-      int cgrid = slots * (int)((2 * C + AMD_TPB - 1) / AMD_TPB);
-      bn_collapse_partials_kernel<<<cgrid, AMD_TPB, 0, stream>>>(
-          sums.data_ptr<float>(), sums2.data_ptr<float>(), rgrid,
-          (int)(2 * C), slots);
-      CHECK_CUDA_OK();
-    }
-    int fgrid = (int)((C + 63) / 64);
-    bn_finalize_train_kernel<<<fgrid, AMD_TPB, 0, stream>>>(
-        sums2.data_ptr<float>(), slots, weight.data_ptr<float>(),
-        bias.data_ptr<float>(), running_mean.data_ptr<float>(),
-        running_var.data_ptr<float>(), mean.data_ptr<float>(),
-        invstd.data_ptr<float>(), scale.data_ptr<float>(),
-        shift.data_ptr<float>(), R, (int)C, (float)momentum, (float)eps);
-    CHECK_CUDA_OK();
     long total_vec = R * C / VEC;
     int agrid = amd_grid(total_vec);
     size_t smem = 2 * C * sizeof(float);
@@ -474,36 +673,15 @@
   check_nhwc(x);
   const long C = x.size(1);
   const long R = x.numel() / C;
-  TORCH_CHECK(parts.size(1) == 2 * C, "parts must be [nparts][2C]");
-  const int nparts = (int)parts.size(0);
-  auto opts = x.options().dtype(at::kFloat);
-  auto mean = at::empty({C}, opts);
-  auto invstd = at::empty({C}, opts);
-  auto scale = at::empty({C}, opts);
-  auto shift = at::empty({C}, opts);
   auto y = at::empty_like(x);
   at::Tensor mask;
   if (relu && addend)
     mask = at::empty({R * C / 4}, x.options().dtype(at::kByte));
   auto stream = at::cuda::getCurrentCUDAStream();
-
-  const int slots = bn_collapse_slots(nparts);
-  auto sums2 = at::empty({slots, 2 * C}, opts);
-  {
-    int cgrid = slots * (int)((2 * C + AMD_TPB - 1) / AMD_TPB);
-    bn_collapse_partials_kernel<<<cgrid, AMD_TPB, 0, stream>>>(
-        parts.data_ptr<float>(), sums2.data_ptr<float>(), nparts,
-        (int)(2 * C), slots);
-    CHECK_CUDA_OK();
-  }
-  int fgrid = (int)((C + 63) / 64);
-  bn_finalize_train_kernel<<<fgrid, AMD_TPB, 0, stream>>>(
-      sums2.data_ptr<float>(), slots, weight.data_ptr<float>(),
-      bias.data_ptr<float>(), running_mean.data_ptr<float>(),
-      running_var.data_ptr<float>(), mean.data_ptr<float>(),
-      invstd.data_ptr<float>(), scale.data_ptr<float>(),
-      shift.data_ptr<float>(), R, (int)C, (float)momentum, (float)eps);
-  CHECK_CUDA_OK();
+  auto st = bn_train_stats(x, parts, weight, bias, running_mean, running_var,
+                           momentum, eps);
+  auto &mean = st.mean, &invstd = st.invstd, &scale = st.scale,
+       &shift = st.shift;
   dispatch_vec(x, [&](auto* tp, auto vec) {
     using devT = std::remove_pointer_t<decltype(tp)>;
     constexpr int VEC = decltype(vec)::value;
@@ -528,6 +706,97 @@
   });
   if (!mask.defined()) mask = at::empty({0}, x.options().dtype(at::kByte));
   return {y, mean, invstd, scale, shift, mask};
+}
+
+std::vector<at::Tensor> batch_norm_dual_fwd_train(
+    at::Tensor x3, at::Tensor x_d, std::optional<at::Tensor> parts3,
+    std::optional<at::Tensor> parts_d, at::Tensor weight3, at::Tensor bias3,
+    at::Tensor running_mean3, at::Tensor running_var3, double momentum3,
+    double eps3, at::Tensor weight_d, at::Tensor bias_d,
+    at::Tensor running_mean_d, at::Tensor running_var_d, double momentum_d,
+    double eps_d) {
+  check_dual(x3, x_d);
+  const long C = x3.size(1);
+  const long R = x3.numel() / C;
+  auto sd = bn_train_stats(x_d, parts_d, weight_d, bias_d, running_mean_d,
+                           running_var_d, momentum_d, eps_d);
+  auto s3 = bn_train_stats(x3, parts3, weight3, bias3, running_mean3,
+                           running_var3, momentum3, eps3);
+  auto y = at::empty_like(x3);
+  auto mask = at::empty({R * C / 4}, x3.options().dtype(at::kByte));
+  auto stream = at::cuda::getCurrentCUDAStream();
+  dispatch_vec(x3, [&](auto* tp, auto vec) {
+    using devT = std::remove_pointer_t<decltype(tp)>;
+    constexpr int VEC = decltype(vec)::value;
+    long total_vec = R * C / VEC;
+    int agrid = amd_grid(total_vec);
+    bn_apply_kernel<devT, VEC, true, true, true, true>
+        <<<agrid, AMD_TPB, 0, stream>>>(
+            (const devT*)x3.const_data_ptr(),
+            (const devT*)x_d.const_data_ptr(), (devT*)y.data_ptr(),
+            mask.data_ptr<unsigned char>(), s3.scale.data_ptr<float>(),
+            s3.shift.data_ptr<float>(), total_vec, (int)C,
+            sd.scale.data_ptr<float>(), sd.shift.data_ptr<float>());
+    CHECK_CUDA_OK();
+  });
+  return {y, s3.mean, s3.invstd, sd.mean, sd.invstd, mask};
+}
+
+std::vector<at::Tensor> batch_norm_dual_bwd(
+    at::Tensor x3, at::Tensor x_d, at::Tensor grad_out,
+    std::optional<at::Tensor> grad_out2, at::Tensor relu_mask,
+    at::Tensor weight3, at::Tensor mean3, at::Tensor invstd3,
+    at::Tensor weight_d, at::Tensor mean_d, at::Tensor invstd_d) {
+  check_dual(x3, x_d);
+  check_nhwc(grad_out);
+  const long C = x3.size(1);
+  const long R = x3.numel() / C;
+  TORCH_CHECK(relu_mask.numel() == R * C / 4, "relu_mask size mismatch");
+  auto opts = x3.options().dtype(at::kFloat);
+  const int rgrid = bn_reduce_grid(R, C);
+  auto sums3 = at::empty({rgrid, 2 * C}, opts);
+  auto sums_d = at::empty({rgrid, 2 * C}, opts);
+  auto ghat = at::empty_like(grad_out);
+  auto gx3 = at::empty_like(x3);
+  auto gx_d = at::empty_like(x_d);
+  BNBwdCoeffs k3, kd;
+  auto stream = at::cuda::getCurrentCUDAStream();
+  dispatch_vec(x3, [&](auto* tp, auto vec) {
+    using devT = std::remove_pointer_t<decltype(tp)>;
+    constexpr int VEC = decltype(vec)::value;
+    const devT* go2p = grad_out2
+        ? (const devT*)grad_out2->const_data_ptr() : nullptr;
+    BNDualSide<devT> rs{(const devT*)x_d.const_data_ptr(),
+                        mean_d.data_ptr<float>(), invstd_d.data_ptr<float>(),
+                        sums_d.data_ptr<float>()};
+#define REDUCE_DUAL(GO2_)                                                   \
+  bn_reduce_kernel<devT, VEC, true, 3, true, GO2_, true>                    \
+      <<<rgrid, AMD_TPB, 0, stream>>>(                                      \
+          (const devT*)x3.const_data_ptr(),                                 \
+          (const devT*)grad_out.const_data_ptr(), go2p,                     \
+          (const devT*)relu_mask.const_data_ptr(), mean3.data_ptr<float>(), \
+          invstd3.data_ptr<float>(), nullptr, nullptr,                      \
+          (devT*)ghat.data_ptr(), sums3.data_ptr<float>(), R, (int)C, rs)
+    if (go2p) REDUCE_DUAL(true);
+    else REDUCE_DUAL(false);
+#undef REDUCE_DUAL
+    CHECK_CUDA_OK();
+    k3 = bn_bwd_coeffs(sums3, weight3, mean3, invstd3, R, C);
+    kd = bn_bwd_coeffs(sums_d, weight_d, mean_d, invstd_d, R, C);
+    long total_vec = R * C / VEC;
+    int agrid = amd_grid(total_vec);
+    BNDualBwdSide<devT> as{(const devT*)x_d.const_data_ptr(),
+                           (devT*)gx_d.data_ptr(), kd.A.data_ptr<float>(),
+                           kd.Bc.data_ptr<float>(), kd.Dc.data_ptr<float>()};
+    bn_bwd_apply_kernel<devT, VEC, 0, false, true, true>
+        <<<agrid, AMD_TPB, 0, stream>>>(
+            (const devT*)x3.const_data_ptr(),
+            (const devT*)ghat.const_data_ptr(), (devT*)gx3.data_ptr(),
+            nullptr, k3.A.data_ptr<float>(), k3.Bc.data_ptr<float>(),
+            k3.Dc.data_ptr<float>(), nullptr, nullptr, total_vec, (int)C, as);
+    CHECK_CUDA_OK();
+  });
+  return {gx3, k3.gw, k3.gb, gx_d, kd.gw, kd.gb};
 }
 
 at::Tensor batch_norm_fwd_eval(at::Tensor x, at::Tensor weight,
@@ -575,7 +844,8 @@
 }
 
 std::vector<at::Tensor> batch_norm_bwd(at::Tensor x, at::Tensor grad_out,
-                                       at::Tensor y, at::Tensor weight,
+                                       std::optional<at::Tensor> y,
+                                       at::Tensor weight,
                                        at::Tensor mean, at::Tensor invstd,
                                        bool relu, bool need_ghat,
                                        std::optional<at::Tensor> scale,
@@ -589,11 +859,7 @@
   auto opts = x.options().dtype(at::kFloat);
   const int rgrid = bn_reduce_grid(R, C);
   auto sums = at::empty({rgrid, 2 * C}, opts);
-  auto gw = at::empty({C}, opts);
-  auto gb = at::empty({C}, opts);
-  auto A = at::empty({C}, opts);
-  auto Bc = at::empty({C}, opts);
-  auto Dc = at::empty({C}, opts);
+  BNBwdCoeffs k;
   auto gx = at::empty_like(x);
   const bool affine_mask = relu && !need_ghat && scale && shift;
   const bool mask_y = relu && (!affine_mask || grad_out2.has_value());
@@ -613,7 +879,7 @@
       <<<rgrid, AMD_TPB, 0, stream>>>(                                      \
           (const devT*)x.const_data_ptr(),                                  \
           (const devT*)grad_out.const_data_ptr(), go2p,                     \
-          (const devT*)y.const_data_ptr(), mean.data_ptr<float>(),          \
+          yp, mean.data_ptr<float>(),                                       \
           invstd.data_ptr<float>(), scp, shp,                               \
           WG_ ? (devT*)ghat.data_ptr() : nullptr,                           \
           sums.data_ptr<float>(), R, (int)C)
@@ -628,6 +894,10 @@
           sums.data_ptr<float>(), R, (int)C)
     const unsigned char* mkp = (relu_mask && relu_mask->numel())
         ? relu_mask->data_ptr<unsigned char>() : nullptr;
+    TORCH_CHECK(y.has_value() || !mask_y || mkp,
+                "batch_norm_bwd: y is required to mask a relu+addend BN "
+                "that saved no relu_mask");
+    const devT* yp = y ? (const devT*)y->const_data_ptr() : nullptr;
     if (mask_y && mkp && go2p) REDUCE3(true);
     else if (mask_y && mkp) REDUCE3(false);
     else if (mask_y && go2p) REDUCE(1, true, true);
@@ -638,22 +908,7 @@
 #undef REDUCE
 #undef REDUCE3
     CHECK_CUDA_OK();
-    const int slots = bn_collapse_slots(rgrid);
-    auto sums2 = at::empty({slots, 2 * C}, opts);
-    {
-      int cgrid = slots * (int)((2 * C + AMD_TPB - 1) / AMD_TPB);
-      bn_collapse_partials_kernel<<<cgrid, AMD_TPB, 0, stream>>>(
-          sums.data_ptr<float>(), sums2.data_ptr<float>(), rgrid,
-          (int)(2 * C), slots);
-      CHECK_CUDA_OK();
-    }
-    int fgrid = (int)((C + 63) / 64);
-    bn_bwd_finalize_kernel<<<fgrid, AMD_TPB, 0, stream>>>(
-        sums2.data_ptr<float>(), slots, weight.data_ptr<float>(),
-        mean.data_ptr<float>(), invstd.data_ptr<float>(),
-        gw.data_ptr<float>(), gb.data_ptr<float>(), A.data_ptr<float>(),
-        Bc.data_ptr<float>(), Dc.data_ptr<float>(), R, (int)C);
-    CHECK_CUDA_OK();
+    k = bn_bwd_coeffs(sums, weight, mean, invstd, R, C);
     long total_vec = R * C / VEC;
     int agrid = amd_grid(total_vec);
     size_t smem = (affine_mask ? 5 : 3) * C * sizeof(float);
@@ -664,13 +919,13 @@
   bn_bwd_apply_kernel<devT, VEC, MASK_, false, true>                        \
       <<<agrid, AMD_TPB, smem, stream>>>(                                   \
           (const devT*)x.const_data_ptr(), go_in, (devT*)gx.data_ptr(),     \
-          nullptr, A.data_ptr<float>(), Bc.data_ptr<float>(),               \
-          Dc.data_ptr<float>(), scp, shp, total_vec, (int)C)
+          nullptr, k.A.data_ptr<float>(), k.Bc.data_ptr<float>(),           \
+          k.Dc.data_ptr<float>(), scp, shp, total_vec, (int)C)
     if (affine_mask) BAPPLY(2);
     else BAPPLY(0);
 #undef BAPPLY
     CHECK_CUDA_OK();
   });
   if (!ghat.defined()) ghat = grad_out;
-  return {gx, gw, gb, ghat};
-}
+  return {gx, k.gw, k.gb, ghat};
+}
diff --git a/amdtrain/ops/csrc/ext.cpp b/amdtrain/ops/csrc/ext.cpp
--- a/amdtrain/ops/csrc/ext.cpp
+++ b/amdtrain/ops/csrc/ext.cpp
@@ -35,8 +35,25 @@
                                at::Tensor bias, at::Tensor running_mean,
                                at::Tensor running_var, double eps, bool relu,
                                std::optional<at::Tensor> addend);
+std::vector<at::Tensor> batch_norm_train_stats(
+    at::Tensor x, std::optional<at::Tensor> parts, at::Tensor weight,
+    at::Tensor bias, at::Tensor running_mean, at::Tensor running_var,
+    double momentum, double eps);
+std::vector<at::Tensor> batch_norm_dual_fwd_train(
+    at::Tensor x3, at::Tensor x_d, std::optional<at::Tensor> parts3,
+    std::optional<at::Tensor> parts_d, at::Tensor weight3, at::Tensor bias3,
+    at::Tensor running_mean3, at::Tensor running_var3, double momentum3,
+    double eps3, at::Tensor weight_d, at::Tensor bias_d,
+    at::Tensor running_mean_d, at::Tensor running_var_d, double momentum_d,
+    double eps_d);
+std::vector<at::Tensor> batch_norm_dual_bwd(
+    at::Tensor x3, at::Tensor x_d, at::Tensor grad_out,
+    std::optional<at::Tensor> grad_out2, at::Tensor relu_mask,
+    at::Tensor weight3, at::Tensor mean3, at::Tensor invstd3,
+    at::Tensor weight_d, at::Tensor mean_d, at::Tensor invstd_d);
 std::vector<at::Tensor> batch_norm_bwd(at::Tensor x, at::Tensor grad_out,
-                                       at::Tensor y, at::Tensor weight,
+                                       std::optional<at::Tensor> y,
+                                       at::Tensor weight,
                                        at::Tensor mean, at::Tensor invstd,
                                        bool relu, bool need_ghat,
                                        std::optional<at::Tensor> scale,
@@ -86,7 +103,9 @@
                               long H, long W, long KH, long KW, long stride,
                               long pad);
 
-std::vector<at::Tensor> max_pool_3x3_s2_fwd(at::Tensor x);
+std::vector<at::Tensor> max_pool_3x3_s2_fwd(at::Tensor x,
+                                            std::optional<at::Tensor> scale,
+                                            std::optional<at::Tensor> shift);
 at::Tensor max_pool_3x3_s2_bwd(at::Tensor grad_y, at::Tensor idx, long H,
                                long W);
 at::Tensor global_avg_pool_fwd(at::Tensor x);
@@ -115,6 +134,9 @@
         py::arg("x"), py::arg("weight"), py::arg("bias"),
         py::arg("running_mean"), py::arg("running_var"), py::arg("eps"),
         py::arg("relu"), py::arg("addend") = std::nullopt);
+  m.def("batch_norm_train_stats", &batch_norm_train_stats);
+  m.def("batch_norm_dual_fwd_train", &batch_norm_dual_fwd_train);
+  m.def("batch_norm_dual_bwd", &batch_norm_dual_bwd);
   m.def("batch_norm_bwd", &batch_norm_bwd, py::arg("x"), py::arg("grad_out"),
         py::arg("y"), py::arg("weight"), py::arg("mean"), py::arg("invstd"),
         py::arg("relu"), py::arg("need_ghat"),
@@ -150,7 +172,8 @@
   m.def("conv_generic_fwd", &conv_generic_fwd);
   m.def("conv_generic_wgrad", &conv_generic_wgrad);
   m.def("conv_generic_dgrad", &conv_generic_dgrad);
-  m.def("max_pool_3x3_s2_fwd", &max_pool_3x3_s2_fwd);
+  m.def("max_pool_3x3_s2_fwd", &max_pool_3x3_s2_fwd, py::arg("x"),
+        py::arg("scale") = std::nullopt, py::arg("shift") = std::nullopt);
   m.def("max_pool_3x3_s2_bwd", &max_pool_3x3_s2_bwd);
   m.def("global_avg_pool_fwd", &global_avg_pool_fwd);
   m.def("global_avg_pool_bwd", &global_avg_pool_bwd);
diff --git a/amdtrain/ops/csrc/pool.hip b/amdtrain/ops/csrc/pool.hip
--- a/amdtrain/ops/csrc/pool.hip
+++ b/amdtrain/ops/csrc/pool.hip
@@ -2,11 +2,21 @@
 
 namespace {
 
-template <typename T, int VEC>
+template <typename T, int VEC, bool BNRELU = false>
 __global__ void __launch_bounds__(AMD_TPB)
 maxpool_fwd_kernel(const T* __restrict__ x, T* __restrict__ y,
                    unsigned char* __restrict__ idx, long N, int H, int W,
-                   int C, int Ho, int Wo) {
+                   int C, int Ho, int Wo,
+                   const float* __restrict__ scale = nullptr,
+                   const float* __restrict__ shift = nullptr) {
+  extern __shared__ float sm[];
+  if (BNRELU) {
+    for (int c = threadIdx.x; c < C; c += blockDim.x) {
+      sm[c] = scale[c];
+      sm[C + c] = shift[c];
+    }
+    __syncthreads();
+  }
   const int gpr = C / VEC;
   const long total = N * Ho * Wo * gpr;
   for (long i = (long)blockIdx.x * blockDim.x + threadIdx.x; i < total;
@@ -39,6 +49,9 @@
 #pragma unroll
         for (int k = 0; k < VEC; ++k) {
           float v = to_f32(xv.v[k]);
+          if (BNRELU)
+            v = to_f32(from_f32<T>(
+                fmaxf(sm[c0 + k] * v + sm[C + c0 + k], 0.f)));
           if (v > best[k]) {
             best[k] = v;
             bidx[k] = (unsigned char)(kh * 3 + kw);
@@ -160,8 +173,18 @@
 
 }
 
-std::vector<at::Tensor> max_pool_3x3_s2_fwd(at::Tensor x) {
+std::vector<at::Tensor> max_pool_3x3_s2_fwd(at::Tensor x,
+                                            std::optional<at::Tensor> scale,
+                                            std::optional<at::Tensor> shift) {
   check_nhwc4(x);
+  TORCH_CHECK(scale.has_value() == shift.has_value(),
+              "scale and shift come together");
+  const bool bnrelu = scale.has_value();
+  if (bnrelu)
+    TORCH_CHECK(scale->numel() == x.size(1) && shift->numel() == x.size(1) &&
+                    scale->scalar_type() == at::kFloat &&
+                    shift->scalar_type() == at::kFloat,
+                "scale/shift must be [C] fp32");
   const long N = x.size(0), C = x.size(1), H = x.size(2), W = x.size(3);
   const long Ho = (H + 2 - 3) / 2 + 1, Wo = (W + 2 - 3) / 2 + 1;
   auto y = at::empty({N, C, Ho, Wo},
@@ -178,11 +201,19 @@
         constexpr int VEC = 16 / sizeof(devT);
         TORCH_CHECK(C % VEC == 0);
         long total = N * Ho * Wo * (C / VEC);
-        maxpool_fwd_kernel<devT, VEC>
-            <<<amd_grid(total), AMD_TPB, 0, stream>>>(
-                (const devT*)x.const_data_ptr(), (devT*)y.data_ptr(),
-                (unsigned char*)idx.data_ptr(), N, (int)H, (int)W, (int)C,
-                (int)Ho, (int)Wo);
+        if (bnrelu)
+          maxpool_fwd_kernel<devT, VEC, true>
+              <<<amd_grid(total), AMD_TPB, 2 * C * sizeof(float), stream>>>(
+                  (const devT*)x.const_data_ptr(), (devT*)y.data_ptr(),
+                  (unsigned char*)idx.data_ptr(), N, (int)H, (int)W, (int)C,
+                  (int)Ho, (int)Wo, scale->data_ptr<float>(),
+                  shift->data_ptr<float>());
+        else
+          maxpool_fwd_kernel<devT, VEC>
+              <<<amd_grid(total), AMD_TPB, 0, stream>>>(
+                  (const devT*)x.const_data_ptr(), (devT*)y.data_ptr(),
+                  (unsigned char*)idx.data_ptr(), N, (int)H, (int)W, (int)C,
+                  (int)Ho, (int)Wo);
         CHECK_CUDA_OK();
       });
   return {y, idx};
diff --git a/amdtrain/ops/fused.py b/amdtrain/ops/fused.py
--- a/amdtrain/ops/fused.py
+++ b/amdtrain/ops/fused.py
@@ -1,6 +1,7 @@
 
 from __future__ import annotations
 
+import os
 from typing import Optional
 
 import torch
@@ -9,7 +10,8 @@
 from ._ext import require_ext, use_ext_for
 from .conv import GradCell
 
-__all__ = ["batch_norm", "bn_add_relu", "max_pool_3x3_s2", "global_avg_pool"]
+__all__ = ["batch_norm", "bn_add_relu", "bn_add_relu_downsample",
+           "bn_relu_max_pool", "max_pool_3x3_s2", "global_avg_pool"]
 
 
 class _BNFunction(torch.autograd.Function):
@@ -92,6 +94,79 @@
     return batch_norm(x, bn, relu=True, addend=addend)
 
 
+class _BNDualFunction(torch.autograd.Function):
+
+    @staticmethod
+    def forward(ctx, x3, x_d, weight3, bias3, running_mean3, running_var3,
+                momentum3, eps3, weight_d, bias_d, running_mean_d,
+                running_var_d, momentum_d, eps_d, parts3, parts_d, res_cell):
+        e = require_ext()
+        y, mean3, invstd3, mean_d, invstd_d, mask = \
+            e.batch_norm_dual_fwd_train(
+                x3, x_d, parts3, parts_d,
+                weight3, bias3, running_mean3, running_var3,
+                float(momentum3), float(eps3),
+                weight_d, bias_d, running_mean_d, running_var_d,
+                float(momentum_d), float(eps_d))
+        ctx.save_for_backward(x3, x_d, weight3, mean3, invstd3, weight_d,
+                              mean_d, invstd_d, mask)
+        ctx.res_cell = res_cell
+        return y
+
+    @staticmethod
+    def backward(ctx, grad_out):
+        (x3, x_d, weight3, mean3, invstd3, weight_d, mean_d, invstd_d,
+         mask) = ctx.saved_tensors
+        e = require_ext()
+        go2 = None
+        cell = getattr(ctx, "res_cell", None)
+        if cell is not None and cell.g is not None:
+            go2 = cell.g.contiguous(memory_format=torch.channels_last)
+            cell.g = None
+        gx3, gw3, gb3, gx_d, gw_d, gb_d = e.batch_norm_dual_bwd(
+            x3, x_d, grad_out.contiguous(memory_format=torch.channels_last),
+            go2, mask, weight3, mean3, invstd3, weight_d, mean_d, invstd_d)
+        return (gx3, gx_d, gw3, gb3, None, None, None, None, gw_d, gb_d,
+                None, None, None, None, None, None, None)
+
+
+def _dsfuse_enabled() -> bool:
+    return os.environ.get("AMDTRAIN_DSFUSE", "1") == "1"
+
+
+def _stemfuse_enabled() -> bool:
+    return os.environ.get("AMDTRAIN_STEMFUSE", "1") == "1"
+
+
+def _vec_ok(x: torch.Tensor, max_groups: int) -> bool:
+    C = x.size(1)
+    vec = 16 // x.element_size()
+    return (C & (C - 1)) == 0 and C % vec == 0 and C // vec <= max_groups
+
+
+def bn_add_relu_downsample(x3: torch.Tensor, bn3, x_d: torch.Tensor,
+                           bn_d) -> torch.Tensor:
+    if (bn3.training and bn_d.training and _dsfuse_enabled()
+            and use_ext_for(x3) and x3.shape == x_d.shape
+            and x3.dtype == x_d.dtype and _vec_ok(x3, 256)):
+        for bn in (bn_d, bn3):
+            if bn.track_running_stats and bn.num_batches_tracked is not None:
+                bn.num_batches_tracked.add_(1)
+        parts3 = getattr(x3, "_amdtrain_bn_stats", None)
+        parts_d = getattr(x_d, "_amdtrain_bn_stats", None)
+        cell = GradCell()
+        out = _BNDualFunction.apply(
+            x3.contiguous(memory_format=torch.channels_last),
+            x_d.contiguous(memory_format=torch.channels_last),
+            bn3.weight, bn3.bias, bn3.running_mean, bn3.running_var,
+            bn3.momentum, bn3.eps, bn_d.weight, bn_d.bias,
+            bn_d.running_mean, bn_d.running_var, bn_d.momentum, bn_d.eps,
+            parts3, parts_d, cell)
+        out._amdtrain_next_cell = cell
+        return out
+    return bn_add_relu(x3, bn3, batch_norm(x_d, bn_d))
+
+
 class _MaxPool3x3S2(torch.autograd.Function):
     @staticmethod
     def forward(ctx, x):
@@ -118,6 +193,45 @@
     return F.max_pool2d(x, kernel_size=3, stride=2, padding=1)
 
 
+class _BNReLUMaxPool(torch.autograd.Function):
+
+    @staticmethod
+    def forward(ctx, x, weight, bias, running_mean, running_var, momentum,
+                eps, parts):
+        e = require_ext()
+        mean, invstd, scale, shift = e.batch_norm_train_stats(
+            x, parts, weight, bias, running_mean, running_var,
+            float(momentum), float(eps))
+        y, idx = e.max_pool_3x3_s2_fwd(x, scale, shift)
+        ctx.save_for_backward(x, idx, weight, mean, invstd, scale, shift)
+        return y
+
+    @staticmethod
+    def backward(ctx, grad_out):
+        x, idx, weight, mean, invstd, scale, shift = ctx.saved_tensors
+        e = require_ext()
+        gp = e.max_pool_3x3_s2_bwd(
+            grad_out.contiguous(memory_format=torch.channels_last), idx,
+            int(x.size(2)), int(x.size(3)))
+        grad_x, grad_w, grad_b, _ = e.batch_norm_bwd(
+            x, gp, None, weight, mean, invstd, True, False, scale, shift,
+            None, None)
+        return grad_x, grad_w, grad_b, None, None, None, None, None
+
+
+def bn_relu_max_pool(x: torch.Tensor, bn) -> torch.Tensor:
+    if (bn.training and _stemfuse_enabled() and use_ext_for(x)
+            and _vec_ok(x, 512)):
+        if bn.track_running_stats and bn.num_batches_tracked is not None:
+            bn.num_batches_tracked.add_(1)
+        parts = getattr(x, "_amdtrain_bn_stats", None)
+        return _BNReLUMaxPool.apply(
+            x.contiguous(memory_format=torch.channels_last), bn.weight,
+            bn.bias, bn.running_mean, bn.running_var, bn.momentum, bn.eps,
+            parts)
+    return max_pool_3x3_s2(batch_norm(x, bn, relu=True))
+
+
 class _GlobalAvgPool(torch.autograd.Function):
     @staticmethod
     def forward(ctx, x):
```

After: 10190 images/sec, median of 6. 3.3% higher.
